# vita-epfl/motion-style-transfer

Measured on AMD Instinct MI355X. Metric: trajectories/sec fwd+bwd (Y-Net+LoRA, SDD shortterm), higher is better.
Workload: dtype f32; 1 GPU; C2: SDD shortterm Y-Net + LoRA rank=1 on encoder[0-4], 256x256 raster, obs=8 pred=12; batch_per_gpu=32, global_batch=32, raster=256x256, obs_len=8, pred_len=12, train_net=mosa_1, parallelism=dp1, trainable_floats=8190

## Files before the change

include/ynet_hip.h:

```cpp
#ifndef YNET_HIP_H
#define YNET_HIP_H

#ifdef __cplusplus
extern "C" {
#endif

int ynet_abi_version(void);
const char* ynet_last_error(void);

long long ynet_packed_weight_floats(int cout, int cin, int K, int mode);
int ynet_pack_weight(const float* w, float* wp, int cout, int cin, int K, int mode, void* stream);

long long ynet_conv2d_workspace_floats(int B, int H, int W, int cout);
int ynet_conv2d(const float* const* src, const int* src_c, const long long* src_bs, const int* src_bmod, int nsrc,
                const float* mask, long long mask_bs, const float* wp, const float* bias,
                float* const* dst, const int* dst_c, const long long* dst_bs, int ndst,
                int B, int H, int W, int K, int relu, float* workspace, long long workspace_floats,
                void* stream);
int ynet_conv2d_pool_supported(int B, int H, int W, int cout, int K);
int ynet_conv2d_pool(const float* const* src, const int* src_c, const long long* src_bs, int nsrc, const float* wp, const float* bias,
                     float* dst, int cout, long long dst_bs, float* pooled, long long pooled_bs,
                     int B, int H, int W, int K, int relu, void* stream);
int ynet_conv2d_dgrad_relu_supported(int B, int H, int W, int dx_c, int K);
int ynet_conv2d_dgrad_relu(const float* dy, int dy_c, long long dy_bs, const float* mask, long long mask_bs, const float* wp,
                           float* dx, int dx_c, long long dx_bs, const float* relu_of, long long relu_of_bs,
                           int B, int H, int W, int K, float* workspace, long long workspace_floats, void* stream);
int ynet_conv2d_add_supported(int B, int H, int W, int cout, int K);
int ynet_conv2d_add(const float* const* src, const int* src_c, const long long* src_bs, const int* src_bmod, int nsrc,
                    const float* wp, const float* bias, float* dst, int cout, long long dst_bs,
                    int B, int H, int W, int K, int relu, const float* addend, long long addend_bs, int addend_bmod,
                    void* stream);

long long ynet_conv2d_relu_bits_words(int B, int H, int W, int cout, int K);
int ynet_conv2d_relu_bits(const float* const* src, const int* src_c, const long long* src_bs, int nsrc, const float* wp, const float* bias,
                          float* dst, int cout, long long dst_bs, unsigned* bits, int B, int H, int W, int K, void* stream);
int ynet_conv2d_dgrad_relu_bits(const float* dy, int dy_c, long long dy_bs, const float* mask, long long mask_bs, const float* wp,
                                float* dx, int dx_c, long long dx_bs, const unsigned* bits, int B, int H, int W, int K, void* stream);

int ynet_conv2d_winograd_supported(int B, int H, int W, int cin, int cout, int K);
long long ynet_winograd_filter_floats(int cin, int cout);
int ynet_winograd_filter(const float* wp, float* u, int cin, int cout, int col0, int cols_total, void* stream);
int ynet_conv2d_winograd(const float* src, long long src_bs, const float* u, const float* bias, float* dst, long long dst_bs, int cin, int cout,
                         int B, int H, int W, int relu, void* stream);
int ynet_conv2d_winograd_s2d(const float* src, long long src_bs, const float* u, float* dst, long long dst_bs, int cin, int cout, int B, int H, int W, void* stream);
int ynet_conv2d_winograd_pred_bce_supported(int B, int H, int W, int cin, int cout, int pred_cout, int kernlen);
int ynet_conv2d_winograd_pred_bce_blob(const float* src, long long src_bs, const float* u, const float* bias, const float* pred_wp, const float* pred_bias, int pred_cout,
                                       const float* target_xy, const float* blob, int kernlen, int S, float* logits, float* loss, float* dx, long long dx_bs,
                                       void* workspace, int B, int H, int W, float expected_grad, void* stream);
int ynet_conv2d_winograd_split_supported(int B, int H, int W, int cin);
int ynet_conv2d_winograd_split(const float* src, long long src_bs, const float* u, float* dst0, long long dst0_bs, int dst0_s2d, float* dst1, long long dst1_bs, int cin,
                               int B, int H, int W, void* stream);
int ynet_conv2d_winograd_dgrad_relu(const float* dy, long long dy_bs, const float* u, float* dx, long long dx_bs, const float* relu_of, long long relu_of_bs,
                                    int dy_c, int dx_c, int B, int H, int W, void* stream);
int ynet_conv2d_winograd_cat_supported(int B, int H, int W, const int* src_c, int nsrc, int cout, int K);
long long ynet_winograd_filter_cat_floats(const int* src_c, int nsrc, int cout);
int ynet_winograd_filter_cat(const float* wp, float* u, const int* src_c, int nsrc, int cout, int col0, int cols_total, void* stream);
int ynet_conv2d_winograd_cat(const float* const* src, const int* src_c, const long long* src_bs, int nsrc, const float* u, const float* bias, float* dst,
                             long long dst_bs, int cout, int B, int H, int W, int relu, void* stream);
int ynet_conv2d_winograd_cat_add(const float* const* src, const int* src_c, const long long* src_bs, int nsrc, const float* u, const float* bias, float* dst,
                                 long long dst_bs, int cout, int B, int H, int W, int relu, const float* addend, long long addend_bs, int addend_bmod,
                                 void* stream);
int ynet_conv2d_winograd_cat_pool(const float* const* src, const int* src_c, const long long* src_bs, int nsrc, const float* u, const float* bias, float* dst,
                                  long long dst_bs, float* pooled, long long pooled_bs, int cout, int B, int H, int W, int relu, void* stream);
int ynet_conv2d_winograd_cat_pool_code(const float* const* src, const int* src_c, const long long* src_bs, int nsrc, const float* u, const float* bias, float* dst,
                                       long long dst_bs, float* pooled, long long pooled_bs, unsigned char* code, int B, int H, int W, void* stream);
long long ynet_winograd_relu_bits_words(int B, int H, int W);
int ynet_conv2d_winograd_relu_bits(const float* src, long long src_bs, const float* u, const float* bias, float* dst, long long dst_bs, int cin, int B, int H, int W,
                                   unsigned* bits_out, void* stream);
int ynet_conv2d_winograd_cat_relu_bits(const float* const* src, const int* src_c, const long long* src_bs, int nsrc, const float* u, const float* bias, float* dst,
                                       long long dst_bs, int B, int H, int W, const float* addend, long long addend_bs, int addend_bmod, unsigned* bits_out,
                                       void* stream);
int ynet_conv2d_winograd_dgrad_relu_bits(const float* dy, long long dy_bs, const float* u, float* dx, long long dx_bs, const unsigned* bits, int dy_c, int B, int H,
                                         int W, void* stream);
int ynet_conv2d_winograd16_supported(int B, int H, int W, const int* src_c, int nsrc, int cout, int K);
long long ynet_winograd16_filter_floats(const int* src_c, int nsrc, int cout);
int ynet_winograd16_filter(const float* wp, float* u, const int* src_c, int nsrc, int cout, int col0, int cols_total, void* stream);
int ynet_conv2d_winograd16(const float* const* src, const int* src_c, const long long* src_bs, int nsrc, const float* u, const float* bias, float* dst,
                           long long dst_bs, int cout, int B, int H, int W, int relu, const float* relu_of, long long relu_of_bs, const float* addend,
                           long long addend_bs, int addend_bmod, float* pooled, long long pooled_bs, void* stream);
int ynet_upsample2x_conv2d_winograd_supported(int B, int H, int W, int cin, int cout, int K);
int ynet_upsample2x_conv2d_winograd(const float* src, long long src_bs, const float* u, const float* bias, float* dst, long long dst_bs, int cin, int cout, int B,
                                    int H, int W, int relu, void* stream);

#define YNET_AUTO_NO_WINOGRAD 1u
#define YNET_AUTO_NO_WINOGRAD16 2u
#define YNET_AUTO_WINOGRAD16_FOR_16 4u
#define YNET_AUTO_NO_POOL_CODE 8u
#define YNET_AUTO_NO_RELU_WBITS 16u
#define YNET_AUTO_NO_SPLIT48 32u
#define YNET_AUTO_UPCONV_BWD 64u
typedef struct YnetConvAuto {
    const float* src[4];
    int src_c[4];
    long long src_bs[4];
    int src_bmod[4];
    int nsrc;
    const float* mask;
    long long mask_bs;
    const float* wp;
    const float* bias;
    float* dst[4];
    int dst_c[4];
    long long dst_bs[4];
    int ndst;
    int B, H, W, K, relu;
    int upsample2x;
    const float* relu_of;
    long long relu_of_bs;
    float* pooled;
    long long pooled_bs;
    unsigned char* pool_code;
    const float* addend;
    long long addend_bs;
    int addend_bmod;
    unsigned* bits_out;
    const unsigned* relu_bits;
    unsigned* wbits_out;
    const unsigned* relu_wbits;
    float* cache;
    long long cache_floats;
    unsigned long long* cache_tag;
    unsigned long long wp_version;
    float* workspace;
    long long workspace_floats;
    unsigned flags;
    int dst_s2d[4];
} YnetConvAuto;
typedef struct YnetConvTaken {
    int family;
    int variant;
    int nlaunch;
    int tmpl[4][3];
    int wrote_wbits, wrote_pool_code, transformed;
    int wrote_s2d;
} YnetConvTaken;
long long ynet_conv2d_auto_cache_floats(const YnetConvAuto* desc);
long long ynet_conv2d_auto_workspace_floats(const YnetConvAuto* desc);
int ynet_conv2d_auto(const YnetConvAuto* desc, YnetConvTaken* taken, void* stream);
int ynet_conv2d_auto_plan(const YnetConvAuto* desc, YnetConvTaken* taken);

long long ynet_upconv_tables_floats(int cout, int cin, long long* keff_floats, long long* table_floats);
int ynet_upconv_tables(const float* w, int cout, int cin, float* keff_packed, float* tables, void* stream);
int ynet_upconv_dgrad_ring(const float* D, long long d_bs, const float* tables, const float* relu_of, long long relu_of_bs, float* dx, long long dx_bs,
                           int B, int C4, int cin, int h, int w, void* stream);

int ynet_conv2d_plan(int B, int H, int W, int cout, int K);

long long ynet_conv2d_wgrad_workspace_floats(int B, int H, int W, int cout, int cin, int K);
int ynet_conv2d_wgrad(const float* const* src, const int* src_c, const long long* src_bs, int nsrc,
                      const float* dy, long long dy_bs, const float* mask, long long mask_bs,
                      float* dw, float* db, float* workspace, int B, int H, int W, int cout, int K,
                      void* stream);

int ynet_lora_compose(const float* w, const float* lora_a, const float* lora_b, float scale, float* w_eff,
                      int cout, int cin, int K, int r, void* stream);
int ynet_lora_grad(const float* dw, const float* lora_a, const float* lora_b, float scale, float* d_a, float* d_b,
                   int cout, int cin, int K, int r, void* stream);

int ynet_lora_compose_pack(const float* w, const float* lora_a, const float* lora_b, float scale, float* wp_fwd,
                           float* wp_dgrad, int cout, int cin, int K, int r, void* stream);
int ynet_lora_compose_pack_multi(int n, const float* const* w, const float* const* lora_a, const float* const* lora_b,
                                 const float* scale, float* const* wp_fwd, float* const* wp_dgrad, const int* cout,
                                 const int* cin, const int* K, const int* r, void* stream);

int ynet_lora_conv2d_wgrad_supported(int cin, int cout, int K, int r, int W);
int ynet_lora_conv2d_wgrad_preferred(int cin, int cout, int K, int r, int W);
long long ynet_lora_conv2d_wgrad_workspace_floats(int cin, int cout);
int ynet_lora_conv2d_wgrad(const float* const* src, const int* src_c, const long long* src_bs, int nsrc,
                           const float* dy, long long dy_batch_stride, const float* mask, long long mask_batch_stride,
                           const float* lora_a, const float* lora_b, float scale, float* d_a, float* d_b,
                           float* workspace, int B, int H, int W, int cout, int K, int r, void* stream);

int ynet_maxpool2_fwd(const float* x, float* y, long long N, int H, int W, void* stream);
int ynet_maxpool2_bwd(const float* x, const float* dy, float* dx, long long N, int H, int W, void* stream);
int ynet_maxpool2_bwd_add(const float* x, const float* dy, const float* add0, const float* add1, float* dx, long long N,
                          int H, int W, int relu_mask, void* stream);
int ynet_maxpool2_bwd_add_code(const unsigned char* code, const float* dy, const float* add0, const float* add1, float* dx, long long N, int H, int W,
                               int relu_mask, void* stream);
int ynet_upsample2x_fwd(const float* x, float* y, long long N, int H, int W, void* stream);
int ynet_upsample2x_bwd(const float* dy, float* dx, long long N, int H, int W, void* stream);
int ynet_upsample2x_bwd_relu(const float* dy, float* dx, const float* relu_of, long long N, int H, int W, void* stream);
int ynet_avgpool_pyramid(const float* x, float* const* outs, int nlev, long long N, int H, int W, void* stream);

long long ynet_batchnorm_workspace_doubles(int C);
int ynet_batchnorm2d_fwd(const float* x, float* y, const float* gamma, const float* beta, float* running_mean, float* running_var, float* save_mean, float* save_invstd,
                         double* workspace, int B, int C, long long HW, int train, double momentum, double eps, void* stream);
int ynet_batchnorm2d_bwd(const float* dy, const float* x, const float* mean, const float* invstd, const float* gamma, float* dx, float* dgamma, float* dbeta, double* workspace,
                         int B, int C, long long HW, int train, void* stream);
int ynet_add_relu(const float* a, const float* b, float* y, long long n, int relu, void* stream);
int ynet_relu_bwd(const float* dy, const float* y, float* dx, long long n, void* stream);

long long ynet_bce_workspace_bytes(void);
int ynet_bce_logits_fwd(const float* x, const float* t, long long n, float* loss, void* workspace, void* stream);
int ynet_bce_logits_bwd(const float* x, const float* t, const float* grad_out, float* dx, long long n, void* stream);
int ynet_bce_logits_fwd_grad(const float* x, const float* t, long long n, float expected_grad, float* loss, float* dx,
                             void* workspace, void* stream);
int ynet_bce_grad_rescale(float* dx, const float* grad_out, float expected_grad, long long n, void* stream);

long long ynet_pred_bce_workspace_bytes(void);
int ynet_pred_bce(const float* x, long long x_batch_stride, const float* wp, const float* bias, const float* target,
                  float* y, float* loss, float* dx, float* dy, void* workspace, int B, int cin, int cout, long long HW,
                  float expected_grad, int dx_relu_mask, void* stream);
int ynet_pred_bce_blob(const float* x, long long x_batch_stride, const float* wp, const float* bias, const float* target_xy, const float* blob, int kernlen,
                       int S, int H, int W, float* y, float* loss, float* dx, float* dy, void* workspace, int B, int cin, int cout, float expected_grad,
                       int dx_relu_mask, void* stream);

int ynet_softargmax2d(const float* x, float* out, long long B, int C, long long batch_stride, int H, int W,
                      void* stream);

// ... 66 lines not shown
```

motion-style-transfer_amd/_lib.py:

```python
import ctypes
import os
import re

_HERE = os.path.dirname(os.path.abspath(__file__))
LIB_PATH = os.environ.get("YNET_HIP_LIB") or os.path.join(_HERE, "csrc", "libynet_hip.so")
HEADER_PATH = os.path.join(os.path.dirname(_HERE), "include", "ynet_hip.h")

c_fp = ctypes.c_void_p
c_i = ctypes.c_int
c_ll = ctypes.c_longlong
c_f = ctypes.c_float
PP = ctypes.POINTER(ctypes.c_void_p)
PI = ctypes.POINTER(ctypes.c_int)
PLL = ctypes.POINTER(ctypes.c_longlong)

class ConvAuto(ctypes.Structure):
    _fields_ = [("src", c_fp * 4), ("src_c", c_i * 4), ("src_bs", c_ll * 4), ("src_bmod", c_i * 4), ("nsrc", c_i),
                ("mask", c_fp), ("mask_bs", c_ll), ("wp", c_fp), ("bias", c_fp),
                ("dst", c_fp * 4), ("dst_c", c_i * 4), ("dst_bs", c_ll * 4), ("ndst", c_i),
                ("B", c_i), ("H", c_i), ("W", c_i), ("K", c_i), ("relu", c_i), ("upsample2x", c_i),
                ("relu_of", c_fp), ("relu_of_bs", c_ll), ("pooled", c_fp), ("pooled_bs", c_ll), ("pool_code", c_fp),
                ("addend", c_fp), ("addend_bs", c_ll), ("addend_bmod", c_i),
                ("bits_out", c_fp), ("relu_bits", c_fp), ("wbits_out", c_fp), ("relu_wbits", c_fp),
                ("cache", c_fp), ("cache_floats", c_ll), ("cache_tag", ctypes.POINTER(ctypes.c_ulonglong)), ("wp_version", ctypes.c_ulonglong),
                ("workspace", c_fp), ("workspace_floats", c_ll), ("flags", ctypes.c_uint), ("dst_s2d", c_i * 4)]


class ConvTaken(ctypes.Structure):
    _fields_ = [("family", c_i), ("variant", c_i), ("nlaunch", c_i), ("tmpl", (c_i * 3) * 4), ("wrote_wbits", c_i), ("wrote_pool_code", c_i),
                ("transformed", c_i), ("wrote_s2d", c_i)]


AUTO_NO_WINOGRAD, AUTO_NO_WINOGRAD16, AUTO_WINOGRAD16_FOR_16, AUTO_NO_POOL_CODE, AUTO_NO_RELU_WBITS, AUTO_NO_SPLIT48 = 1, 2, 4, 8, 16, 32
AUTO_UPCONV_BWD = 64

SIGNATURES = {
    "ynet_abi_version": (c_i, []),
    "ynet_last_error": (ctypes.c_char_p, []),
    "ynet_packed_weight_floats": (c_ll, [c_i, c_i, c_i, c_i]),
    "ynet_pack_weight": (c_i, [c_fp, c_fp, c_i, c_i, c_i, c_i, c_fp]),
    "ynet_conv2d_workspace_floats": (c_ll, [c_i, c_i, c_i, c_i]),
    "ynet_conv2d": (c_i, [PP, PI, PLL, PI, c_i, c_fp, c_ll, c_fp, c_fp, PP, PI, PLL, c_i,
                          c_i, c_i, c_i, c_i, c_i, c_fp, c_ll, c_fp]),
    "ynet_conv2d_pool_supported": (c_i, [c_i, c_i, c_i, c_i, c_i]),
    "ynet_conv2d_pool": (c_i, [PP, PI, PLL, c_i, c_fp, c_fp, c_fp, c_i, c_ll, c_fp, c_ll, c_i, c_i, c_i, c_i, c_i, c_fp]),
    "ynet_conv2d_dgrad_relu_supported": (c_i, [c_i, c_i, c_i, c_i, c_i]),
    "ynet_conv2d_dgrad_relu": (c_i, [c_fp, c_i, c_ll, c_fp, c_ll, c_fp, c_fp, c_i, c_ll, c_fp, c_ll, c_i, c_i, c_i, c_i, c_fp, c_ll, c_fp]),
    "ynet_conv2d_relu_bits_words": (c_ll, [c_i, c_i, c_i, c_i, c_i]),
    "ynet_conv2d_relu_bits": (c_i, [PP, PI, PLL, c_i, c_fp, c_fp, c_fp, c_i, c_ll, c_fp, c_i, c_i, c_i, c_i, c_fp]),
    "ynet_conv2d_dgrad_relu_bits": (c_i, [c_fp, c_i, c_ll, c_fp, c_ll, c_fp, c_fp, c_i, c_ll, c_fp, c_i, c_i, c_i, c_i, c_fp]),
    "ynet_conv2d_winograd_supported": (c_i, [c_i, c_i, c_i, c_i, c_i, c_i]),
    "ynet_winograd_filter_floats": (c_ll, [c_i, c_i]),
    "ynet_winograd_filter": (c_i, [c_fp, c_fp, c_i, c_i, c_i, c_i, c_fp]),
    "ynet_conv2d_winograd": (c_i, [c_fp, c_ll, c_fp, c_fp, c_fp, c_ll, c_i, c_i, c_i, c_i, c_i, c_i, c_fp]),
    "ynet_conv2d_winograd_s2d": (c_i, [c_fp, c_ll, c_fp, c_fp, c_ll, c_i, c_i, c_i, c_i, c_i, c_fp]),
    "ynet_conv2d_winograd_pred_bce_supported": (c_i, [c_i, c_i, c_i, c_i, c_i, c_i, c_i]),
    "ynet_conv2d_winograd_pred_bce_blob": (c_i, [c_fp, c_ll, c_fp, c_fp, c_fp, c_fp, c_i, c_fp, c_fp, c_i, c_i, c_fp, c_fp, c_fp, c_ll, c_fp, c_i, c_i, c_i,
                                                 c_f, c_fp]),
    "ynet_conv2d_winograd_split_supported": (c_i, [c_i, c_i, c_i, c_i]),
    "ynet_conv2d_winograd_split": (c_i, [c_fp, c_ll, c_fp, c_fp, c_ll, c_i, c_fp, c_ll, c_i, c_i, c_i, c_i, c_fp]),
    "ynet_upconv_dgrad_ring": (c_i, [c_fp, c_ll, c_fp, c_fp, c_ll, c_fp, c_ll, c_i, c_i, c_i, c_i, c_i, c_fp]),
    "ynet_upconv_tables_floats": (c_ll, [c_i, c_i, PLL, PLL]),
    "ynet_upconv_tables": (c_i, [c_fp, c_i, c_i, c_fp, c_fp, c_fp]),
    "ynet_conv2d_winograd_dgrad_relu": (c_i, [c_fp, c_ll, c_fp, c_fp, c_ll, c_fp, c_ll, c_i, c_i, c_i, c_i, c_i, c_fp]),
    "ynet_conv2d_winograd_cat_supported": (c_i, [c_i, c_i, c_i, PI, c_i, c_i, c_i]),
    "ynet_winograd_filter_cat_floats": (c_ll, [PI, c_i, c_i]),
    "ynet_winograd_filter_cat": (c_i, [c_fp, c_fp, PI, c_i, c_i, c_i, c_i, c_fp]),
    "ynet_conv2d_winograd_cat": (c_i, [PP, PI, PLL, c_i, c_fp, c_fp, c_fp, c_ll, c_i, c_i, c_i, c_i, c_i, c_fp]),
    "ynet_conv2d_winograd_cat_add": (c_i, [PP, PI, PLL, c_i, c_fp, c_fp, c_fp, c_ll, c_i, c_i, c_i, c_i, c_i, c_fp, c_ll, c_i, c_fp]),
    "ynet_conv2d_winograd_cat_pool": (c_i, [PP, PI, PLL, c_i, c_fp, c_fp, c_fp, c_ll, c_fp, c_ll, c_i, c_i, c_i, c_i, c_i, c_fp]),
    "ynet_conv2d_winograd_cat_pool_code": (c_i, [PP, PI, PLL, c_i, c_fp, c_fp, c_fp, c_ll, c_fp, c_ll, c_fp, c_i, c_i, c_i, c_fp]),
    "ynet_winograd_relu_bits_words": (c_ll, [c_i, c_i, c_i]),
    "ynet_conv2d_winograd_relu_bits": (c_i, [c_fp, c_ll, c_fp, c_fp, c_fp, c_ll, c_i, c_i, c_i, c_i, c_fp, c_fp]),
    "ynet_conv2d_winograd_cat_relu_bits": (c_i, [PP, PI, PLL, c_i, c_fp, c_fp, c_fp, c_ll, c_i, c_i, c_i, c_fp, c_ll, c_i, c_fp, c_fp]),
    "ynet_conv2d_winograd_dgrad_relu_bits": (c_i, [c_fp, c_ll, c_fp, c_fp, c_ll, c_fp, c_i, c_i, c_i, c_i, c_fp]),
    "ynet_upsample2x_conv2d_winograd_supported": (c_i, [c_i, c_i, c_i, c_i, c_i, c_i]),
    "ynet_upsample2x_conv2d_winograd": (c_i, [c_fp, c_ll, c_fp, c_fp, c_fp, c_ll, c_i, c_i, c_i, c_i, c_i, c_i, c_fp]),
    "ynet_conv2d_winograd16_supported": (c_i, [c_i, c_i, c_i, PI, c_i, c_i, c_i]),
    "ynet_winograd16_filter_floats": (c_ll, [PI, c_i, c_i]),
    "ynet_winograd16_filter": (c_i, [c_fp, c_fp, PI, c_i, c_i, c_i, c_i, c_fp]),
    "ynet_conv2d_winograd16": (c_i, [PP, PI, PLL, c_i, c_fp, c_fp, c_fp, c_ll, c_i, c_i, c_i, c_i, c_i, c_fp, c_ll, c_fp, c_ll, c_i, c_fp, c_ll, c_fp]),
    "ynet_conv2d_auto_cache_floats": (c_ll, [ctypes.POINTER(ConvAuto)]),
    "ynet_conv2d_auto_workspace_floats": (c_ll, [ctypes.POINTER(ConvAuto)]),
    "ynet_conv2d_auto": (c_i, [ctypes.POINTER(ConvAuto), ctypes.POINTER(ConvTaken), c_fp]),
    "ynet_conv2d_auto_plan": (c_i, [ctypes.POINTER(ConvAuto), ctypes.POINTER(ConvTaken)]),
    "ynet_conv2d_add_supported": (c_i, [c_i, c_i, c_i, c_i, c_i]),
    "ynet_conv2d_add": (c_i, [PP, PI, PLL, PI, c_i, c_fp, c_fp, c_fp, c_i, c_ll, c_i, c_i, c_i, c_i, c_i, c_fp, c_ll, c_i, c_fp]),
    "ynet_conv2d_plan": (c_i, [c_i, c_i, c_i, c_i, c_i]),
    "ynet_conv2d_wgrad_workspace_floats": (c_ll, [c_i, c_i, c_i, c_i, c_i, c_i]),
    "ynet_conv2d_wgrad": (c_i, [PP, PI, PLL, c_i, c_fp, c_ll, c_fp, c_ll, c_fp, c_fp, c_fp,
                                c_i, c_i, c_i, c_i, c_i, c_fp]),
    "ynet_lora_compose": (c_i, [c_fp, c_fp, c_fp, c_f, c_fp, c_i, c_i, c_i, c_i, c_fp]),
    "ynet_lora_grad": (c_i, [c_fp, c_fp, c_fp, c_f, c_fp, c_fp, c_i, c_i, c_i, c_i, c_fp]),
    "ynet_lora_conv2d_wgrad_supported": (c_i, [c_i, c_i, c_i, c_i, c_i]),
    "ynet_lora_conv2d_wgrad_preferred": (c_i, [c_i, c_i, c_i, c_i, c_i]),
    "ynet_lora_conv2d_wgrad_workspace_floats": (c_ll, [c_i, c_i]),
    "ynet_lora_conv2d_wgrad": (c_i, [PP, PI, PLL, c_i, c_fp, c_ll, c_fp, c_ll, c_fp, c_fp, c_f, c_fp, c_fp, c_fp,
                                     c_i, c_i, c_i, c_i, c_i, c_i, c_fp]),
    "ynet_lora_compose_pack": (c_i, [c_fp, c_fp, c_fp, c_f, c_fp, c_fp, c_i, c_i, c_i, c_i, c_fp]),
    "ynet_lora_compose_pack_multi": (c_i, [c_i, PP, PP, PP, ctypes.POINTER(c_f), PP, PP, PI, PI, PI, PI, c_fp]),
    "ynet_batch_sum": (c_i, [c_fp, c_fp, c_i, c_ll, c_ll, c_fp]),
    "ynet_adam_step": (c_i, [c_fp, c_fp, c_fp, c_i, c_i, ctypes.c_double, ctypes.c_double, ctypes.c_double, ctypes.c_double, ctypes.c_double,
                             c_i, c_fp]),
    "ynet_maxpool2_fwd": (c_i, [c_fp, c_fp, c_ll, c_i, c_i, c_fp]),
    "ynet_maxpool2_bwd": (c_i, [c_fp, c_fp, c_fp, c_ll, c_i, c_i, c_fp]),
    "ynet_maxpool2_bwd_add": (c_i, [c_fp, c_fp, c_fp, c_fp, c_fp, c_ll, c_i, c_i, c_i, c_fp]),
    "ynet_maxpool2_bwd_add_code": (c_i, [c_fp, c_fp, c_fp, c_fp, c_fp, c_ll, c_i, c_i, c_i, c_fp]),
    "ynet_upsample2x_fwd": (c_i, [c_fp, c_fp, c_ll, c_i, c_i, c_fp]),
    "ynet_upsample2x_bwd": (c_i, [c_fp, c_fp, c_ll, c_i, c_i, c_fp]),
    "ynet_upsample2x_bwd_relu": (c_i, [c_fp, c_fp, c_fp, c_ll, c_i, c_i, c_fp]),
    "ynet_avgpool_pyramid": (c_i, [c_fp, PP, c_i, c_ll, c_i, c_i, c_fp]),
    "ynet_bce_workspace_bytes": (c_ll, []),
    "ynet_bce_logits_fwd": (c_i, [c_fp, c_fp, c_ll, c_fp, c_fp, c_fp]),
    "ynet_bce_logits_bwd": (c_i, [c_fp, c_fp, c_fp, c_fp, c_ll, c_fp]),
    "ynet_bce_logits_fwd_grad": (c_i, [c_fp, c_fp, c_ll, c_f, c_fp, c_fp, c_fp, c_fp]),
    "ynet_bce_grad_rescale": (c_i, [c_fp, c_fp, c_f, c_ll, c_fp]),
    "ynet_pred_bce_workspace_bytes": (c_ll, []),
    "ynet_pred_bce": (c_i, [c_fp, c_ll, c_fp, c_fp, c_fp, c_fp, c_fp, c_fp, c_fp, c_fp, c_i, c_i, c_i, c_ll, c_f, c_i, c_fp]),
    "ynet_pred_bce_blob": (c_i, [c_fp, c_ll, c_fp, c_fp, c_fp, c_fp, c_i, c_i, c_i, c_i, c_fp, c_fp, c_fp, c_fp, c_fp, c_i, c_i, c_i, c_f, c_i, c_fp]),
    "ynet_softargmax2d": (c_i, [c_fp, c_fp, c_ll, c_i, c_ll, c_i, c_i, c_fp]),
    "ynet_train_readout": (c_i, [c_fp, c_ll, c_fp, c_ll, c_i, c_fp, c_fp, c_fp, c_fp, c_fp, c_i, c_i, c_i, c_i, c_f, c_fp]),
    "ynet_pred_softargmax_supported": (c_i, [c_i, c_i, c_i, c_i]),
    "ynet_pred_softargmax_workspace_floats": (c_ll, [c_ll, c_i, c_i]),
    "ynet_pred_softargmax": (c_i, [c_fp, c_ll, c_fp, c_fp, c_fp, c_fp, c_ll, c_i, c_i, c_i, c_i, c_fp]),
    "ynet_pad2d": (c_i, [c_fp, c_fp, c_ll, c_i, c_i, c_i, c_i, c_fp]),
    "ynet_seg_onehot_pad": (c_i, [c_fp, c_fp, c_i, c_i, c_i, c_i, c_i, c_fp]),
    "ynet_resize_nearest": (c_i, [c_fp, c_fp, c_i, c_i, c_i, c_i, ctypes.c_double, ctypes.c_double, c_fp]),
    "ynet_batchnorm_workspace_doubles": (c_ll, [c_i]),
    "ynet_batchnorm2d_fwd": (c_i, [c_fp] * 9 + [c_i, c_i, c_ll, c_i, ctypes.c_double, ctypes.c_double, c_fp]),
    "ynet_batchnorm2d_bwd": (c_i, [c_fp] * 9 + [c_i, c_i, c_ll, c_i, c_fp]),
    "ynet_add_relu": (c_i, [c_fp, c_fp, c_fp, c_ll, c_i, c_fp]),
    "ynet_relu_bwd": (c_i, [c_fp, c_fp, c_fp, c_ll, c_fp]),
    "ynet_rot90_flip": (c_i, [c_fp, c_fp, c_ll, c_i, c_i, c_i, c_i, c_fp]),
    "ynet_rot_coords": (c_i, [c_fp, c_ll] + [ctypes.c_double] * 8 + [c_fp]),
    "ynet_sigmoid_temp": (c_i, [c_fp, c_fp, c_ll, c_i, c_ll, PI, c_i, c_f, c_fp]),
    "ynet_gather_patch": (c_i, [c_fp, c_i, c_i, c_fp, c_fp, c_i, c_i, c_i, c_fp, c_fp]),
    "ynet_heatmap_analytic": (c_i, [c_fp, c_fp, c_i, c_i, c_i, c_i, c_i, ctypes.c_double, c_fp, c_i, c_fp, c_fp]),
    "ynet_kmeans2d": (c_i, [c_fp, c_fp, c_fp, c_fp, c_i, c_i, c_i, ctypes.c_float, c_i, c_fp]),
    "ynet_comm_handle_bytes": (c_ll, []),
    "ynet_comm_create": (c_i, [c_i, c_i, c_ll, PP]),
    "ynet_comm_export": (c_i, [c_fp, c_fp]),
    "ynet_comm_connect": (c_i, [c_fp, c_fp]),
    "ynet_allreduce_sum": (c_i, [c_fp, c_fp, c_ll, c_fp]),
    "ynet_comm_status": (c_i, [c_fp]),
    "ynet_comm_destroy": (c_i, [c_fp]),
    "ynet_multinomial": (c_i, [c_fp, c_ll, c_ll, c_i, c_i, c_i, c_f, ctypes.c_ulonglong, c_fp, c_fp, c_fp]),
    "ynet_multinomial_devseed": (c_i, [c_fp, c_ll, c_ll, c_i, c_i, c_i, c_f, c_fp, c_fp, c_fp, c_fp]),
    "ynet_cws_prior": (c_i, [c_fp, c_ll, c_i, c_fp, c_fp, c_i, c_i, c_i, c_f, c_f, c_i, c_fp, c_fp, c_fp]),
    "ynet_score_rank_samples": (c_i, [c_fp, c_fp, c_fp, c_i, c_i, c_i, c_i, c_i, c_i, c_f, c_fp, c_fp, c_fp, c_fp, c_fp, c_fp]),
    "ynet_score_rank_samples_rows": (c_i, [c_fp, c_fp, c_fp, c_fp, c_i, c_i, c_i, c_i, c_i, c_i, c_f, c_fp, c_fp, c_fp, c_fp, c_fp, c_fp]),
    "ynet_gather_rows": (c_i, [c_fp, c_ll, c_fp, c_fp, c_ll, c_i, c_fp, c_fp]),
    "ynet_input_grad_supported": (c_i, [c_i, c_i, c_i, c_i, c_i, c_i]),
    "ynet_input_grad_workspace_floats": (c_ll, [c_i, c_i, c_i, c_i]),
    "ynet_input_grad": (c_i, [c_fp, c_fp, c_fp, c_fp, c_fp, c_fp, c_i, c_i, c_i, c_i, c_i, c_i, c_fp]),
# ... 40 lines not shown
```

motion-style-transfer_amd/csrc/conv_auto.cpp:

```cpp
#include "ynet_common.h"
#include "../../include/ynet_hip.h"
#include <stdint.h>
#include <string.h>

namespace {

struct Piece {
    float* ptr;
    int n;
    long long bs;
    int col0;
    int dst;
    int whole;
};

enum Kind { K_NONE = 0, K_WINO = 1, K_CAT = 2, K_W16 = 3 };

struct Launch {
    int kind;
    int row0;
    int cs[4], ncs;
    int cout, col0, ctot;
    long long floats;
    long long offset;
// ... 17 lines not shown
        case K_CAT: return ynet_winograd_filter_cat_floats(q.cs, q.ncs, q.cout);
        case K_W16: return ynet_winograd16_filter_floats(q.cs, q.ncs, q.cout);
    }
    return 0;
}

void add_launch(Plan& p, int kind, int row0, const int* cs, int ncs, int cout, int col0, int ctot) {
    Launch& q = p.l[p.nl++];
    q.kind = kind;
    q.row0 = row0;
    q.ncs = ncs;
    for (int i = 0; i < 4; ++i) q.cs[i] = i < ncs ? cs[i] : 0;
    q.cout = cout;
    q.col0 = col0;
    q.ctot = ctot;
    q.floats = (filter_floats(q) + 3) & ~3ll;
    q.offset = p.cache_floats;
    p.cache_floats += q.floats;
}

bool w16_ok(const YnetConvAuto* a, const int* cs, int ncs, int cout) {
    return !(a->flags & (YNET_AUTO_NO_WINOGRAD | YNET_AUTO_NO_WINOGRAD16)) && a->K == 3 && ncs >= 1 && ncs <= 3 &&
           ynet_conv2d_winograd16_supported(a->B, a->H, a->W, cs, ncs, cout, a->K);
}

bool srcs_plain(const YnetConvAuto* a) {
    for (int i = 0; i < a->nsrc; ++i)
        if (a->src_bmod[i] > 0) return false;
    return true;
}

bool srcs_aligned(const YnetConvAuto* a) {
    for (int i = 0; i < a->nsrc; ++i)
        if (!al(a->src[i], 16) || (a->src_bs[i] & 3)) return false;
    return true;
}

int make_plan(const YnetConvAuto* a, Plan& p) {
    memset(&p, 0, sizeof(p));
    const bool wino = !(a->flags & YNET_AUTO_NO_WINOGRAD) && a->K == 3 && srcs_plain(a);
    const int B = a->B, H = a->H, W = a->W, K = a->K;
    int cs[4];
    for (int i = 0; i < 4; ++i) cs[i] = i < a->nsrc ? a->src_c[i] : 0;
    int ctot = 0;
    for (int i = 0; i < a->ndst; ++i) ctot += a->dst_c[i];

    if (a->upsample2x) {
        YNET_REQUIRE(a->nsrc == 1 && a->ndst == 1 && !a->mask && !a->relu_of && !a->pooled && !a->addend && !a->bits_out && !a->relu_bits && !a->wbits_out && !a->relu_wbits,
                     "conv2d_auto: upsample2x takes one source, one destination and no other epilogue operand");
        const int s = wino && al(a->src[0], 16) ? ynet_upsample2x_conv2d_winograd_supported(B, H, W, cs[0], ctot, K) : 0;
        YNET_REQUIRE(s == 1 || s == 2, "conv2d_auto: upsample2x + conv is not served for cin %d cout %d at %dx%d (B %d): run ynet_upsample2x_fwd, then the convolution", cs[0], ctot, H, W, B);
        p.family = s == 1 ? 4 : 5;
        add_launch(p, s == 1 ? K_WINO : K_W16, 0, cs, 1, ctot, 0, ctot);
        return 0;
    }
    if (a->bits_out || a->relu_bits) {
        p.family = 0;
        p.variant = a->bits_out ? 1 : 2;
        return 0;
    }
    if (a->addend) {
        YNET_REQUIRE(a->ndst == 1 && !a->mask && !a->relu_of && !a->pooled, "conv2d_auto: addend takes one destination and no mask / relu_of / pooled");
        const bool ok = !(a->flags & YNET_AUTO_NO_WINOGRAD) && K == 3 && srcs_aligned(a) && al(a->addend, 8) && al(a->dst[0], 8) && !(a->dst_bs[0] & 1) && a->nsrc <= 3;
        bool plain = true;
        for (int i = 0; i < a->nsrc; ++i) plain = plain && a->src_bmod[i] <= 0;
        if (ok && plain && ctot == 32 && ynet_conv2d_winograd_cat_supported(B, H, W, cs, a->nsrc, ctot, K)) {
            p.family = 2;
            p.variant = 30;
            add_launch(p, K_CAT, 0, cs, a->nsrc, ctot, 0, ctot);
        } else if (ok && plain && w16_ok(a, cs, a->nsrc, ctot)) {
            p.family = 3;
            p.variant = 31;
            add_launch(p, K_W16, 0, cs, a->nsrc, ctot, 0, ctot);
        } else {
            YNET_REQUIRE(ynet_conv2d_add_supported(B, H, W, ctot, K), "conv2d_auto: a convolution with an additive term is not served at %dx%d (B %d, cout %d, K %d)", H, W, B, ctot, K);
            p.family = 0;
            p.variant = 32;
        }
        return 0;
    }
    if (a->pooled) {
        YNET_REQUIRE(a->ndst == 1 && !a->mask && !a->relu_of, "conv2d_auto: pooled is for a forward convolution with one destination");
        const bool okp = wino && srcs_aligned(a) && al(a->dst[0], 8) && !(a->dst_bs[0] & 1) && a->nsrc <= 3;
        if (okp && ctot == 32 && ynet_conv2d_winograd_cat_supported(B, H, W, cs, a->nsrc, 32, K)) {
            p.family = 2;
            p.variant = 10;
            add_launch(p, K_CAT, 0, cs, a->nsrc, 32, 0, 32);
        } else if (okp && w16_ok(a, cs, a->nsrc, ctot)) {
            p.family = 3;
            p.variant = 11;
            add_launch(p, K_W16, 0, cs, a->nsrc, ctot, 0, ctot);
        } else {
            p.family = 0;
            p.variant = 12;
        }
        return 0;
    }
    if (wino && !a->mask && a->nsrc == 1 && al(a->src[0], 16) && !(a->src_bs[0] & 3) && (!a->relu_of || (al(a->relu_of, 8) && !(a->relu_of_bs & 1)))) {
        const int cin = cs[0];
        const long long HW = (long long)H * W;
        Piece pieces[8];
        int np = 0, c0 = 0;
        bool pieces_ok = true;
        for (int i = 0; i < a->ndst && pieces_ok; ++i) {
            if (!a->dst[i]) { c0 += a->dst_c[i]; continue; }
            int o = 0;
            const int c = a->dst_c[i];
            while (c - o >= 16 && (c - o) % 16 == 0 && np < 8) {
                const int n = c - o >= 32 ? 32 : 16;
                pieces[np++] = Piece{a->dst[i] + o * HW, n, a->dst_bs[i], c0 + o, i, n == c ? 1 : 0};
                o += n;
            }
            if (o != c) pieces_ok = false;
            c0 += c;
        }
        if (!pieces_ok) np = 0;
        auto piece_al = [&](int cnt) {
            for (int i = 0; i < cnt; ++i)
                if (!al(pieces[i].ptr, 8) || (pieces[i].bs & 1)) return false;
            return true;
        };
        if ((a->flags & YNET_AUTO_WINOGRAD16_FOR_16) && np == 1 && pieces[0].n == 16 && piece_al(1) && w16_ok(a, cs, 1, 16)) {
            p.family = 3;
            p.variant = 20;
            p.pieces[0] = pieces[0];
            p.npieces = 1;
            add_launch(p, K_W16, 0, cs, 1, 16, pieces[0].col0, ctot);
            return 0;
        }
        bool wide = false;
        for (int i = 0; i < a->ndst; ++i) wide = wide || (a->dst[i] && a->dst_c[i] >= 64);
        bool all_sup = np > 0 && np <= (a->relu_of ? 1 : 2) && piece_al(np);
        for (int i = 0; i < np && all_sup; ++i) all_sup = ynet_conv2d_winograd_supported(B, H, W, cin, pieces[i].n, K) != 0;
        if (all_sup && !wide && np == 2 && !a->relu_of && !a->bias && !a->relu && !(a->flags & YNET_AUTO_NO_SPLIT48) && pieces[0].n == 16 && pieces[0].whole &&
            pieces[1].n == 32 && pieces[1].whole && pieces[1].col0 == pieces[0].col0 + 16 && ynet_conv2d_winograd_split_supported(B, H, W, cin)) {
            p.family = 1;
            p.variant = 23;
            p.npieces = 2;
            p.pieces[0] = pieces[0];
            p.pieces[1] = pieces[1];
            add_launch(p, K_WINO, 0, cs, 1, 48, pieces[0].col0, ctot);
            return 0;
        }
        if (all_sup && !wide) {
            p.family = 1;
            p.variant = 21;
            p.npieces = np;
            for (int i = 0; i < np; ++i) {
                p.pieces[i] = pieces[i];
                add_launch(p, K_WINO, 0, cs, 1, pieces[i].n, pieces[i].col0, ctot);
            }
            return 0;
        }
        Piece wanted[4];
        int nw = 0;
        c0 = 0;
        for (int i = 0; i < a->ndst; ++i) {
            if (a->dst[i]) wanted[nw++] = Piece{a->dst[i], a->dst_c[i], a->dst_bs[i], c0, i, 1};
            c0 += a->dst_c[i];
        }
        bool w_ok = nw > 0 && (!a->relu_of || nw == 1);
        for (int i = 0; i < nw && w_ok; ++i) w_ok = al(wanted[i].ptr, 8) && !(wanted[i].bs & 1) && w16_ok(a, cs, 1, wanted[i].n);
        if (w_ok) {
            p.family = 3;
            p.variant = 22;
            p.npieces = nw;
// ... 174 lines not shown
        if (a->cache_tag[0] != sig || a->cache_tag[1] != a->wp_version) {
            if (int rc = transform(a, p, stream)) return rc;
            a->cache_tag[0] = sig;
            a->cache_tag[1] = a->wp_version;
            t.transformed = 1;
        }
    }
    return run_plan(a, p, t, taken, stream);
}

}

namespace {

int run_plan(const YnetConvAuto* a, const Plan& p, YnetConvTaken t, YnetConvTaken* taken, void* stream) {
    const int B = a->B, H = a->H, W = a->W, K = a->K, relu = a->relu ? 1 : 0;
    int ctot = 0;
    for (int i = 0; i < a->ndst; ++i) ctot += a->dst_c[i];
    const float* u0 = p.nl ? a->cache + p.l[0].offset : nullptr;
    const float* u1 = p.nl > 1 ? a->cache + p.l[1].offset : nullptr;
    auto done = [&](int rc) {
        if (!rc && taken) *taken = t;
        return rc;
    };
    auto tag = [&](int i, int x, int y, int z) {
        if (i < 4) { t.tmpl[i][0] = x; t.tmpl[i][1] = y; t.tmpl[i][2] = z; }
        t.nlaunch = i + 1;
    };
    float* ws = a->workspace_floats > 0 ? a->workspace : nullptr;
    const long long nws = ws ? a->workspace_floats : 0;

    switch (p.family) {
    case 4:
    case 5:
        tag(0, p.family == 4 ? 4 : 0, 0, 0);
        return done(ynet_upsample2x_conv2d_winograd(a->src[0], a->src_bs[0], u0, a->bias, a->dst[0], a->dst_bs[0], a->src_c[0], ctot, B, H, W, relu, stream));
    case 1: {
        if (p.variant == 23) {
            const Piece &q0 = p.pieces[0], &q1 = p.pieces[1];
            const int s2d = a->dst_s2d[q0.dst] ? 1 : 0;
            const int rc = ynet_conv2d_winograd_split(a->src[0], a->src_bs[0], u0, q0.ptr, q0.bs, s2d, q1.ptr, q1.bs, a->src_c[0], B, H, W, stream);
            if (rc) return rc;
            if (s2d) t.wrote_s2d |= 1 << q0.dst;
            tag(0, 3, a->src_c[0] / 8, s2d ? 6 : 5);
            return done(0);
        }
        const bool one32 = p.npieces == 1 && p.pieces[0].n == 32;
        unsigned* wb_out = (one32 && relu && !a->relu_of && !(a->flags & YNET_AUTO_NO_RELU_WBITS)) ? a->wbits_out : nullptr;
        const unsigned* wb_in = (one32 && a->relu_of && !relu && !a->bias && !(a->flags & YNET_AUTO_NO_RELU_WBITS)) ? a->relu_wbits : nullptr;
        const int em = wb_out ? 3 : (wb_in ? 2 : (a->relu_of ? 1 : 0));
        for (int i = 0; i < p.npieces; ++i) {
            const Piece& q = p.pieces[i];
            const float* u = a->cache + p.l[i].offset;
            const float* bias = a->bias ? a->bias + q.col0 : nullptr;
            int rc;
            const bool s2d = a->dst_s2d[q.dst] && q.whole && em == 0 && !a->bias && !relu;
            if (s2d) {
                rc = ynet_conv2d_winograd_s2d(a->src[0], a->src_bs[0], u, q.ptr, q.bs, a->src_c[0], q.n, B, H, W, stream);
                if (rc) return rc;
                t.wrote_s2d |= 1 << q.dst;
                tag(i, q.n / 16, a->src_c[0] / 8, 4);
                continue;
            }
            if (wb_out) rc = ynet_conv2d_winograd_relu_bits(a->src[0], a->src_bs[0], u, bias, q.ptr, q.bs, a->src_c[0], B, H, W, wb_out, stream);
            else if (wb_in) rc = ynet_conv2d_winograd_dgrad_relu_bits(a->src[0], a->src_bs[0], u, q.ptr, q.bs, wb_in, a->src_c[0], B, H, W, stream);
            else if (a->relu_of) {
                YNET_REQUIRE(!a->bias && !relu, "conv2d_auto: relu_of is for a data gradient (no bias, no ReLU)");
                rc = ynet_conv2d_winograd_dgrad_relu(a->src[0], a->src_bs[0], u, q.ptr, q.bs, a->relu_of, a->relu_of_bs, a->src_c[0], q.n, B, H, W, stream);
            } else rc = ynet_conv2d_winograd(a->src[0], a->src_bs[0], u, bias, q.ptr, q.bs, a->src_c[0], q.n, B, H, W, relu, stream);
            if (rc) return rc;
            tag(i, q.n / 16, a->src_c[0] / 8, em);
        }
        t.wrote_wbits = wb_out ? 1 : 0;
        return done(0);
    }
    case 2: {
        if (p.variant == 30) {
            unsigned* wb = (relu && !(a->flags & YNET_AUTO_NO_RELU_WBITS)) ? a->wbits_out : nullptr;
            tag(0, 2, wb ? 5 : 2, 0);
            t.wrote_wbits = wb ? 1 : 0;
            if (wb) return done(ynet_conv2d_winograd_cat_relu_bits(a->src, a->src_c, a->src_bs, a->nsrc, u0, a->bias, a->dst[0], a->dst_bs[0], B, H, W, a->addend, a->addend_bs, a->addend_bmod, wb, stream));
            return done(ynet_conv2d_winograd_cat_add(a->src, a->src_c, a->src_bs, a->nsrc, u0, a->bias, a->dst[0], a->dst_bs[0], 32, B, H, W, relu, a->addend, a->addend_bs, a->addend_bmod, stream));
        }
        if (p.variant == 10) {
            unsigned char* code = (relu && !(a->flags & YNET_AUTO_NO_POOL_CODE)) ? a->pool_code : nullptr;
            tag(0, 2, code ? 6 : 3, 0);
            t.wrote_pool_code = code ? 1 : 0;
            if (code) return done(ynet_conv2d_winograd_cat_pool_code(a->src, a->src_c, a->src_bs, a->nsrc, u0, a->bias, a->dst[0], a->dst_bs[0], a->pooled, a->pooled_bs, code, B, H, W, stream));
            return done(ynet_conv2d_winograd_cat_pool(a->src, a->src_c, a->src_bs, a->nsrc, u0, a->bias, a->dst[0], a->dst_bs[0], a->pooled, a->pooled_bs, 32, B, H, W, relu, stream));
        }
        unsigned* wb = (relu && !(a->flags & YNET_AUTO_NO_RELU_WBITS)) ? a->wbits_out : nullptr;
        t.wrote_wbits = wb ? 1 : 0;
        if (p.variant == 40) {
            const long long HW = (long long)H * W;
            int rc = ynet_conv2d_winograd(a->src[0], a->src_bs[0], u0, nullptr, a->dst[0], a->dst_bs[0], 32, 32, B, H, W, 0, stream);
            if (rc) return rc;
            const float* rs[4];
            int rc_[4], nr = 0;
            long long rb[4];
            if (a->src_c[0] > 32) { rs[nr] = a->src[0] + 32 * HW; rc_[nr] = a->src_c[0] - 32; rb[nr] = a->src_bs[0]; ++nr; }
            for (int i = 1; i < a->nsrc; ++i) { rs[nr] = a->src[i]; rc_[nr] = a->src_c[i]; rb[nr] = a->src_bs[i]; ++nr; }
            tag(0, 2, 4, 0);
            tag(1, 2, wb ? 5 : 2, 0);
            if (wb) return done(ynet_conv2d_winograd_cat_relu_bits(rs, rc_, rb, nr, u1, a->bias, a->dst[0], a->dst_bs[0], B, H, W, a->dst[0], a->dst_bs[0], 0, wb, stream));
            return done(ynet_conv2d_winograd_cat_add(rs, rc_, rb, nr, u1, a->bias, a->dst[0], a->dst_bs[0], 32, B, H, W, relu, a->dst[0], a->dst_bs[0], 0, stream));
        }
        tag(0, 2, wb ? 4 : 0, 0);
        if (wb) return done(ynet_conv2d_winograd_cat_relu_bits(a->src, a->src_c, a->src_bs, a->nsrc, u0, a->bias, a->dst[0], a->dst_bs[0], B, H, W, nullptr, 0, 0, wb, stream));
        return done(ynet_conv2d_winograd_cat(a->src, a->src_c, a->src_bs, a->nsrc, u0, a->bias, a->dst[0], a->dst_bs[0], 32, B, H, W, relu, stream));
    }
    case 3: {
        if (p.variant == 31) {
            tag(0, 2, 0, 0);
            return done(ynet_conv2d_winograd16(a->src, a->src_c, a->src_bs, a->nsrc, u0, a->bias, a->dst[0], a->dst_bs[0], ctot, B, H, W, relu, nullptr, 0, a->addend, a->addend_bs,
                                               a->addend_bmod, nullptr, 0, stream));
        }
        if (p.variant == 11) {
            tag(0, 3, 0, 0);
            return done(ynet_conv2d_winograd16(a->src, a->src_c, a->src_bs, a->nsrc, u0, a->bias, a->dst[0], a->dst_bs[0], ctot, B, H, W, relu, nullptr, 0, nullptr, 0, 0, a->pooled,
                                               a->pooled_bs, stream));
        }
        if (p.variant == 20 || p.variant == 22) {
            for (int i = 0; i < p.npieces; ++i) {
                const Piece& q = p.pieces[i];
                if (a->relu_of) YNET_REQUIRE(!a->bias && !relu, "conv2d_auto: relu_of is for a data gradient (no bias, no ReLU)");
                int rc = ynet_conv2d_winograd16(a->src, a->src_c, a->src_bs, 1, a->cache + p.l[i].offset, a->bias ? a->bias + q.col0 : nullptr, q.ptr, q.bs, q.n, B, H, W, relu, a->relu_of,
                                                a->relu_of_bs, nullptr, 0, 0, nullptr, 0, stream);
                if (rc) return rc;
                tag(i, a->relu_of ? 1 : 0, 0, 0);
            }
            return done(0);
        }
        if (p.variant == 43) {
            const int cut = p.pieces[0].col0;
            int rc = ynet_conv2d_winograd16(a->src, a->src_c, a->src_bs, cut, u0, nullptr, a->dst[0], a->dst_bs[0], ctot, B, H, W, 0, nullptr, 0, nullptr, 0, 0, nullptr, 0, stream);
            if (rc) return rc;
            tag(0, 0, 0, 0);
            tag(1, 2, 0, 0);
            return done(ynet_conv2d_winograd16(a->src + cut, a->src_c + cut, a->src_bs + cut, a->nsrc - cut, u1, a->bias, a->dst[0], a->dst_bs[0], ctot, B, H, W, relu, nullptr, 0, a->dst[0],
                                               a->dst_bs[0], 0, nullptr, 0, stream));
        }
        tag(0, 0, 0, 0);
        return done(ynet_conv2d_winograd16(a->src, a->src_c, a->src_bs, a->nsrc, u0, a->bias, a->dst[0], a->dst_bs[0], ctot, B, H, W, relu, nullptr, 0, nullptr, 0, 0, nullptr, 0, stream));
    }
    default: break;
    }
    t.nlaunch = 1;
    const int* bmod = nullptr;
    for (int i = 0; i < a->nsrc; ++i)
        if (a->src_bmod[i] > 0) bmod = a->src_bmod;
    switch (p.variant) {
    case 1:
        YNET_REQUIRE(a->ndst == 1 && !a->mask && !a->relu_of && !a->pooled && relu && !bmod, "conv2d_auto: bits_out is for a forward ReLU convolution with one destination");
        return done(ynet_conv2d_relu_bits(a->src, a->src_c, a->src_bs, a->nsrc, a->wp, a->bias, a->dst[0], a->dst_c[0], a->dst_bs[0], a->bits_out, B, H, W, K, stream));
    case 2:
        YNET_REQUIRE(a->nsrc == 1 && a->ndst == 1 && !a->bias && !relu && !a->relu_of, "conv2d_auto: relu_bits is for a data gradient with one source and one destination");
        return done(ynet_conv2d_dgrad_relu_bits(a->src[0], a->src_c[0], a->src_bs[0], a->mask, a->mask_bs, a->wp, a->dst[0], a->dst_c[0], a->dst_bs[0], a->relu_bits, B, H, W, K, stream));
    case 12:
        YNET_REQUIRE(!bmod, "conv2d_auto: pooled takes no batch modulus");
        return done(ynet_conv2d_pool(a->src, a->src_c, a->src_bs, a->nsrc, a->wp, a->bias, a->dst[0], a->dst_c[0], a->dst_bs[0], a->pooled, a->pooled_bs, B, H, W, K, relu, stream));
    case 32:
        return done(ynet_conv2d_add(a->src, a->src_c, a->src_bs, bmod, a->nsrc, a->wp, a->bias, a->dst[0], ctot, a->dst_bs[0], B, H, W, K, relu, a->addend, a->addend_bs, a->addend_bmod, stream));
    case 3:
        YNET_REQUIRE(a->nsrc == 1 && a->ndst == 1 && !a->bias && !relu, "conv2d_auto: relu_of is for a data gradient with one source and one destination");
        return done(ynet_conv2d_dgrad_relu(a->src[0], a->src_c[0], a->src_bs[0], a->mask, a->mask_bs, a->wp, a->dst[0], a->dst_c[0], a->dst_bs[0], a->relu_of, a->relu_of_bs, B, H, W, K, ws,
                                           nws, stream));
// ... 71 lines not shown
```

motion-style-transfer_amd/csrc/conv_wino.hip:

```cpp
#include "ynet_common.h"
#include "bce_element.h"
#include <math.h>
#include <stdlib.h>
#include <type_traits>

typedef float f32x2 __attribute__((ext_vector_type(2)));
typedef unsigned u32x2 __attribute__((ext_vector_type(2)));
typedef __attribute__((address_space(3))) void* lds_ptr_t;

#define WN_TH 16
#define WN_TW 32
#define WN_LQ 10
#define WN_ROWF 40
#define WN_PLANE_F 160
#define WN_SLOT_BYTES (320 * 16 + 16)
#define WN_RING_BYTES (2 * WN_SLOT_BYTES)
#define WN_THREADS 512

struct WinoArgs {
    const float* x;
    const f32x4* u;
    const float* bias;
    float* y;
    long long x_bs, y_bs;
    int B, H, W, relu, ntiles;
    const float* emask;
    long long emask_bs;
    unsigned* wbits;
    float* y2;
    long long y2_bs;
    const float* pw;
    const float* pb;
    int pco, pco_pad;
    const float* t_xy;
    const float* t_blob;
    int t_m, t_S;
    float* logits;
    double* partial;
    unsigned* ticket;
    float* loss;
    long long n_loss;
    float gs;
};

__device__ __forceinline__ f32x2 wn_v01(f32x2 tl, f32x2 th) {
    f32x2 r;
    asm("v_pk_add_f32 %0, %1, %2 op_sel_hi:[1,0] neg_lo:[0,1]" : "=v"(r) : "v"(tl), "v"(th));
    return r;
}
__device__ __forceinline__ f32x2 wn_v23(f32x2 tl, f32x2 th) {
    f32x2 r;
    asm("v_pk_add_f32 %0, %1, %2 op_sel:[1,0] op_sel_hi:[1,1] neg_lo:[1,0] neg_hi:[0,1]" : "=v"(r) : "v"(tl), "v"(th));
    return r;
}

template <int NCB, int EPI, int BITS = 0, bool S2D = false, int CB0 = 0, int CB1 = NCB>
__device__ __forceinline__ void wino_epilogue(f32x4 (&acc)[16][NCB], const f32x2 (&bias2)[NCB][2], float floor_v, __amdgpu_buffer_rsrc_t ry,
                                              __amdgpu_buffer_rsrc_t rm, unsigned st0, unsigned st1, unsigned so_t, unsigned sm_t, int HW, unsigned stp = 0,
                                              unsigned* wbits = nullptr, unsigned char* pcode = nullptr) {
    unsigned word = 0u;
    if constexpr (BITS == 2) word = *wbits;
#pragma unroll
    for (int cb = CB0; cb < CB1; ++cb) {
        constexpr int NB = CB1 - CB0;
        const int cd = cb - CB0;
        u32x2 mk[2][2][2];
        if constexpr (EPI == 1 || EPI == 2) {
#pragma unroll
            for (int h = 0; h < 2; ++h)
#pragma unroll
                for (int k = 0; k < 2; ++k) {
                    const unsigned sm = sm_t + (unsigned)((cd * 16 + 2 * h + k) * HW * 4);
                    mk[h][k][0] = __builtin_amdgcn_raw_buffer_load_b64(rm, st0, sm, 0);
                    mk[h][k][1] = __builtin_amdgcn_raw_buffer_load_b64(rm, st1, sm, 0);
                }
        }
#pragma unroll
        for (int h = 0; h < 2; ++h) {
            f32x2 m[16];
#pragma unroll
            for (int e = 0; e < 16; ++e)
                m[e] = h == 0 ? __builtin_shufflevector(acc[e][cb], acc[e][cb], 0, 1) : __builtin_shufflevector(acc[e][cb], acc[e][cb], 2, 3);
            m[5] = m[5] + bias2[cb][h];
            f32x2 r0[4], r1[4];
#pragma unroll
            for (int j = 0; j < 4; ++j) {
                r0[j] = m[j] + m[4 + j] + m[8 + j];
                r1[j] = m[4 + j] - m[8 + j] - m[12 + j];
            }
            const f32x2 o00 = r0[0] + r0[1] + r0[2], o01 = r0[1] - r0[2] - r0[3];
            const f32x2 o10 = r1[0] + r1[1] + r1[2], o11 = r1[1] - r1[2] - r1[3];
#pragma unroll
            for (int k = 0; k < 2; ++k) {
                f32x2 row0 = {o00[k], o01[k]}, row1 = {o10[k], o11[k]};
                if constexpr (EPI == 2) {
                    row0 += __builtin_bit_cast(f32x2, mk[h][k][0]);
                    row1 += __builtin_bit_cast(f32x2, mk[h][k][1]);
                }
                row0 = f32x2{row0[0] < floor_v ? floor_v : row0[0], row0[1] < floor_v ? floor_v : row0[1]};
                row1 = f32x2{row1[0] < floor_v ? floor_v : row1[0], row1[1] < floor_v ? floor_v : row1[1]};
                if constexpr (EPI == 1) {
                    const f32x2 m0 = __builtin_bit_cast(f32x2, mk[h][k][0]), m1 = __builtin_bit_cast(f32x2, mk[h][k][1]);
                    row0 = f32x2{m0[0] > 0.f ? row0[0] : 0.f, m0[1] > 0.f ? row0[1] : 0.f};
                    row1 = f32x2{m1[0] > 0.f ? row1[0] : 0.f, m1[1] > 0.f ? row1[1] : 0.f};
                }
                const int bit0 = ((cb * 2 + h) * 2 + k) * 4;
                if constexpr (BITS == 2) {
                    row0 = f32x2{(word >> bit0) & 1u ? row0[0] : 0.f, (word >> (bit0 + 1)) & 1u ? row0[1] : 0.f};
                    row1 = f32x2{(word >> (bit0 + 2)) & 1u ? row1[0] : 0.f, (word >> (bit0 + 3)) & 1u ? row1[1] : 0.f};
                }
                if constexpr (BITS == 1)
                    word |= (row0[0] > 0.f ? 1u << bit0 : 0u) | (row0[1] > 0.f ? 2u << bit0 : 0u) | (row1[0] > 0.f ? 4u << bit0 : 0u) | (row1[1] > 0.f ? 8u << bit0 : 0u);
                if constexpr (S2D) {
                    const unsigned hw = (unsigned)(HW >> 2), ph = (unsigned)(NB * 16) * hw * 4u;
                    const unsigned sc = so_t + (unsigned)(cd * 16 + 2 * h + k) * hw * 4u;
                    const float e00 = row0[0], e01 = row0[1], e10 = row1[0], e11 = row1[1];
                    const bool odd = __lane_id() & 1u;
                    const float g0 = __builtin_bit_cast(float, __builtin_amdgcn_update_dpp(0, __builtin_bit_cast(int, odd ? e00 : e01), 0xB1, 0xF, 0xF, false));
                    const float g1 = __builtin_bit_cast(float, __builtin_amdgcn_update_dpp(0, __builtin_bit_cast(int, odd ? e10 : e11), 0xB1, 0xF, 0xF, false));
                    const f32x2 p0 = odd ? f32x2{g0, e01} : f32x2{e00, g0}, p1 = odd ? f32x2{g1, e11} : f32x2{e10, g1};
                    const unsigned vo = st0 + (odd ? ph - 4u : 0u);
                    __builtin_amdgcn_raw_buffer_store_b64(__builtin_bit_cast(u32x2, p0), ry, vo, sc, 0);
                    __builtin_amdgcn_raw_buffer_store_b64(__builtin_bit_cast(u32x2, p1), ry, vo, sc + 2u * ph, 0);
                    continue;
                }
                const unsigned so = so_t + (unsigned)((cd * 16 + 2 * h + k) * HW * 4);
                __builtin_amdgcn_raw_buffer_store_b64(__builtin_bit_cast(u32x2, row0), ry, st0, so, 0);
                __builtin_amdgcn_raw_buffer_store_b64(__builtin_bit_cast(u32x2, row1), ry, st1, so, 0);
                if constexpr (EPI == 3) {
                    float pm = fmaxf(fmaxf(row0[0], row0[1]), fmaxf(row1[0], row1[1]));
                    if (__builtin_isunordered(row0[0], row0[1]) || __builtin_isunordered(row1[0], row1[1])) pm = __builtin_nanf("");
                    __builtin_amdgcn_raw_buffer_store_b32(__builtin_bit_cast(unsigned, pm), rm, stp, sm_t + (unsigned)((cd * 16 + 2 * h + k) * (HW >> 2) * 4), 0);
                    if constexpr (BITS == 3) {
                        float mx = row0[0];
                        unsigned arg = 0u;
                        if (row0[1] > mx || row0[1] != row0[1]) { mx = row0[1]; arg = 1u; }
                        if (row1[0] > mx || row1[0] != row1[0]) { mx = row1[0]; arg = 2u; }
                        if (row1[1] > mx || row1[1] != row1[1]) { mx = row1[1]; arg = 3u; }
                        const unsigned code = arg | (row0[0] > 0.f ? 4u : 0u) | (row0[1] > 0.f ? 8u : 0u) | (row1[0] > 0.f ? 16u : 0u) | (row1[1] > 0.f ? 32u : 0u);
                        pcode[(cd * 16 + 2 * h + k) * (HW >> 2)] = (unsigned char)code;
                    }
                }
            }
        }
    }
    if constexpr (BITS == 1) *wbits = word;
}

template <int MB, typename PosT>
__device__ __forceinline__ float wino_epilogue_pred(f32x4 (&acc)[16][2], const f32x2 (&bias2)[2][2], const f32x4* tab,
                                                    const WinoArgs& a, __amdgpu_buffer_rsrc_t rdx, __amdgpu_buffer_rsrc_t rlog, unsigned st_rm, unsigned so_rm, int b,
                                                    int py0, int px0, int kq, int H, int W, const float* blob_tab, const PosT* pos_lds) {
    const int HW = H * W;
    float yv[2][4][4];
#pragma unroll
    for (int cb = 0; cb < 2; ++cb)
#pragma unroll
        for (int h = 0; h < 2; ++h) {
            f32x2 m[16];
#pragma unroll
            for (int e = 0; e < 16; ++e)
                m[e] = h == 0 ? __builtin_shufflevector(acc[e][cb], acc[e][cb], 0, 1) : __builtin_shufflevector(acc[e][cb], acc[e][cb], 2, 3);
            m[5] = m[5] + bias2[cb][h];
            f32x2 r0[4], r1[4];
#pragma unroll
            for (int j = 0; j < 4; ++j) {
                r0[j] = m[j] + m[4 + j] + m[8 + j];
                r1[j] = m[4 + j] - m[8 + j] - m[12 + j];
            }
            const f32x2 o00 = r0[0] + r0[1] + r0[2], o01 = r0[1] - r0[2] - r0[3];
            const f32x2 o10 = r1[0] + r1[1] + r1[2], o11 = r1[1] - r1[2] - r1[3];
#pragma unroll
            for (int k = 0; k < 2; ++k) {
                const float v00 = o00[k], v01 = o01[k], v10 = o10[k], v11 = o11[k];
                yv[cb][2 * h + k][0] = v00 < 0.f ? 0.f : v00;
                yv[cb][2 * h + k][1] = v01 < 0.f ? 0.f : v01;
                yv[cb][2 * h + k][2] = v10 < 0.f ? 0.f : v10;
                yv[cb][2 * h + k][3] = v11 < 0.f ? 0.f : v11;
            }
        }
    const unsigned st1 = st_rm + (unsigned)(W * 4);
    float s = 0.f;
    f32x4 dx[2][4];
#pragma unroll
    for (int cb = 0; cb < 2; ++cb)
#pragma unroll
        for (int p = 0; p < 4; ++p) dx[cb][p] = f32x4{0.f, 0.f, 0.f, 0.f};
    auto block = [&](const int mb) {
        f32x4 z[4], dz[4];
        {
            const f32x4 pbv = tab[(4 * MB + mb) * 64];
#pragma unroll
            for (int p = 0; p < 4; ++p) z[p] = pbv;
        }
#pragma unroll
        for (int cb = 0; cb < 2; ++cb) {
            const f32x4 wa = tab[(mb * 2 + cb) * 64];
#pragma unroll
            for (int j = 0; j < 4; ++j)
#pragma unroll
                for (int p = 0; p < 4; ++p) z[p] = __builtin_amdgcn_mfma_f32_16x16x4f32(wa[j], yv[cb][j][p], z[p], 0, 0, 0);
        }
#pragma unroll
        for (int i = 0; i < 4; ++i) {
            const int o = 16 * mb + 4 * kq + i;
            const bool valid = o < a.pco;
            const int rx = valid ? (int)pos_lds[2 * (b * a.pco + o)] : 32767, ry = valid ? (int)pos_lds[2 * (b * a.pco + o) + 1] : 32767;
#pragma unroll
            for (int p = 0; p < 4; ++p) {
                const int by = py0 + (p >> 1) - ry + a.t_m / 2, bx = px0 + (p & 1) - rx + a.t_m / 2;
#if defined(YNET_PRED_EPI_DIAG) && (YNET_PRED_EPI_DIAG & 2)
                const float t = 0.f;
#else
                const float t = (by >= 0 && by < a.t_m && bx >= 0 && bx < a.t_m) ? blob_tab[by * a.t_m + bx] : 0.f;
#endif
                float de;
#if defined(YNET_PRED_EPI_DIAG) && (YNET_PRED_EPI_DIAG & 1)
                de = (z[p][i] - t) * a.gs;
                const float l = z[p][i] - t;
#else
                const float l = bce_element<true, true>(z[p][i], t, a.gs, de);
#endif
                s += valid ? l : 0.f;
                dz[p][i] = valid ? de : 0.f;
            }
        }
#pragma unroll
        for (int i = 0; i < 4; ++i) {
            const f32x2 row0 = {z[0][i], z[1][i]}, row1 = {z[2][i], z[3][i]};
            const unsigned so = so_rm + (unsigned)((16 * mb + i) * HW * 4);
            __builtin_amdgcn_raw_buffer_store_b64(__builtin_bit_cast(u32x2, row0), rlog, st_rm, so, 0);
// ... 265 lines not shown
                cur = nxt;
                if (cur < total_units) nxt = next_unit();
                continue;
            }
            if constexpr (EM == 5 || EM == 6) {
                static_assert(EM < 5 || NCB == 3, "the two-destination epilogue is the 48-channel launch's");
                const __amdgpu_buffer_rsrc_t r0 = __builtin_amdgcn_make_buffer_rsrc(a.y + (long long)b * a.y_bs, 0, (unsigned)(16 * HW * 4), 0x00020000);
                const __amdgpu_buffer_rsrc_t r1 = __builtin_amdgcn_make_buffer_rsrc(a.y2 + (long long)b * a.y2_bs, 0, (unsigned)(32 * HW * 4), 0x00020000);
                if constexpr (EM == 6) wino_epilogue<NCB, 0, 0, true, 0, 1>(acc, bias2, floor_v, r0, r0, st_s2d, st_s2d, so_s2d, so_s2d, HW);
                else wino_epilogue<NCB, 0, 0, false, 0, 1>(acc, bias2, floor_v, r0, r0, st_rm, st_rm + (unsigned)(W * 4), so_rm, so_rm, HW);
                wino_epilogue<NCB, 0, 0, false, 1, 3>(acc, bias2, floor_v, r1, r1, st_rm, st_rm + (unsigned)(W * 4), so_rm, so_rm, HW);
                cur = nxt;
                if (cur < total_units) nxt = next_unit();
                continue;
            }
            const unsigned so_t = EM == 4 ? so_s2d : so_rm;
            const __amdgpu_buffer_rsrc_t ry = __builtin_amdgcn_make_buffer_rsrc(a.y + (long long)b * a.y_bs, 0, y_img, 0x00020000);
            const __amdgpu_buffer_rsrc_t rm =
                __builtin_amdgcn_make_buffer_rsrc(const_cast<float*>(EM == 1 ? a.emask + (long long)b * a.emask_bs : a.y), 0, y_img, 0x00020000);
            unsigned* wb = (EM == 2 || EM == 3) ? a.wbits + (((long long)b * (H >> 1) + (ty * (WN_TH / 2) + (cur & 7))) * tiles_x + tx) * 64 + lane : nullptr;
            wino_epilogue<NCB, EM == 1 ? 1 : 0, EM == 2 ? 2 : (EM == 3 ? 1 : 0), EM == 4>(acc, bias2, floor_v, ry, rm, st0, st1, so_t, so_t, HW, 0, wb);
        }
        cur = nxt;
        if (cur < total_units) nxt = next_unit();
    }
    if constexpr (EM == 7 || EM == 8) {
        double* wsd = reinterpret_cast<double*>(ptab + 5 * PMB * 64);
        unsigned* last = reinterpret_cast<unsigned*>(wsd + NW);
#pragma unroll
        for (int o = 32; o > 0; o >>= 1) acc_loss += __shfl_xor(acc_loss, o, 64);
        if (lane == 0) wsd[wave] = acc_loss;
        __syncthreads();
        if (tid == 0) {
            double t = 0.0;
            for (int i = 0; i < NW; ++i) t += wsd[i];
            a.partial[blockIdx.x] = t;
            __threadfence();
            *last = (atomicAdd(a.ticket, 1u) == gridDim.x - 1) ? 1u : 0u;
        }
        __syncthreads();
        if (*last) {
            __threadfence();
            double t = 0.0;
            for (unsigned i = tid; i < gridDim.x; i += NT) t += ((volatile double*)a.partial)[i];
#pragma unroll
            for (int o = 32; o > 0; o >>= 1) t += __shfl_xor(t, o, 64);
            if (lane == 0) wsd[wave] = t;
            __syncthreads();
            if (tid == 0) {
                double tt = 0.0;
                for (int i = 0; i < NW; ++i) tt += wsd[i];
                a.loss[0] = (float)(tt / (double)a.n_loss);
                *a.ticket = 0u;
            }
        }
    }
}

#define WC_SLOT_BYTES (160 * 16 + 16)
#define WC_RING_BYTES (2 * WC_SLOT_BYTES)
#define WC_MAX_SRC 3

struct WinoCatArgs {
    const float* x[WC_MAX_SRC];
    long long x_bs[WC_MAX_SRC];
    int x_c[WC_MAX_SRC];
    int nsrc, nchunks;
    const f32x4* u;
    const float* bias;
    float* y;
    long long y_bs;
    int B, H, W, relu, ntiles;
    const float* addend;
    long long addend_bs;
    int addend_bmod;
    float* pool;
    long long pool_bs;
    unsigned char* pcode;
    unsigned* wbits;
};

template <int NCB, int EPI_>
__global__ __launch_bounds__(WN_THREADS, 1) void conv_wino_cat_kernel(const WinoCatArgs a) {
    constexpr int EPI = EPI_ == 4 ? 0 : (EPI_ == 5 ? 2 : (EPI_ == 6 ? 3 : EPI_));
    constexpr int BITS = EPI_ == 6 ? 3 : (EPI_ >= 4 ? 1 : 0);
    constexpr bool ADD = EPI == 2;
    extern __shared__ f32x4 smem[];
    constexpr int WQ = 4 * NCB * 64;
    const int tid = threadIdx.x, lane = tid & 63;
    const int wave = __builtin_amdgcn_readfirstlane(tid >> 6);
    const int H = a.H, W = a.W, HW = H * W, nchunks = a.nchunks;
    const int tiles_x = W / WN_TW, tiles_y = H / WN_TH;
    const unsigned lds0 = __builtin_amdgcn_readfirstlane((unsigned)(uintptr_t)smem);
    const unsigned wbytes = (unsigned)(nchunks * WQ * 16);
    const unsigned ring0 = lds0 + wbytes + (unsigned)(wave * WC_RING_BYTES);

    unsigned rel[3], edge[3], planeof[3];
#pragma unroll
    for (int j = 0; j < 3; ++j) {
        const int u = j * 64 + lane, plane = u / 40, rem = u - plane * 40, r = rem / WN_LQ, xq = rem - r * WN_LQ;
        rel[j] = (unsigned)((plane * HW + r * W + 4 * xq) * 4);
        edge[j] = (r == 0 ? 1u : 0u) | (r == 3 ? 2u : 0u) | (xq == 0 ? 4u : 0u) | (xq == WN_LQ - 1 ? 8u : 0u);
        planeof[j] = (unsigned)plane;
    }
    const unsigned lead = (unsigned)((W + 4) * 4);
    const __amdgpu_buffer_rsrc_t ru = __builtin_amdgcn_make_buffer_rsrc(const_cast<f32x4*>(a.u), 0, wbytes, 0x00020000);
    const unsigned y_img = (unsigned)(NCB * 16 * HW * 4);

    const bool xcd_walk = (gridDim.x & 7) == 0 && a.ntiles >= (int)gridDim.x;
    const int per_xcd = (a.ntiles + 7) >> 3;
    const int gstride = xcd_walk ? (int)(gridDim.x >> 3) : (int)gridDim.x;
    const int tile_first = xcd_walk ? (int)(blockIdx.x & 7) * per_xcd + (int)(blockIdx.x >> 3) : (int)blockIdx.x;
    const int tile_end = xcd_walk ? min(a.ntiles, ((int)(blockIdx.x & 7) + 1) * per_xcd) : a.ntiles;
    if (tile_first >= tile_end) return;
    const int my_tiles = (tile_end - tile_first + gstride - 1) / gstride;
    const int total_units = my_tiles * 8;

    const int n = lane & 15, kq = lane >> 4;
    const float floor_v = a.relu ? 0.f : -INFINITY;
    f32x2 bias2[NCB][2];
#pragma unroll
    for (int cb = 0; cb < NCB; ++cb)
#pragma unroll
        for (int h = 0; h < 2; ++h)
            bias2[cb][h] = a.bias ? f32x2{a.bias[cb * 16 + 4 * kq + 2 * h], a.bias[cb * 16 + 4 * kq + 2 * h + 1]} : f32x2{0.f, 0.f};
    asm volatile("s_waitcnt vmcnt(0)" ::: "memory");
#pragma unroll
    for (int cb = 0; cb < NCB; ++cb)
#pragma unroll
        for (int h = 0; h < 2; ++h) asm volatile("" : "+v"(bias2[cb][h]));
    const unsigned st0 = (unsigned)((4 * kq * HW + 2 * n) * 4), st1 = st0 + (unsigned)(W * 4);
    const unsigned stp = (unsigned)((4 * kq * (HW >> 2) + n) * 4);

    for (int j = 0; j < nchunks * WQ / WN_THREADS; ++j)
        __builtin_amdgcn_raw_ptr_buffer_load_lds(ru, (lds_ptr_t)(uintptr_t)(lds0 + (unsigned)(j * 8192 + wave * 1024)), 16,
                                                 (unsigned)((j * WN_THREADS + tid) * 16), 0, 0, 0);
    unsigned* unit_ctr = reinterpret_cast<unsigned*>(reinterpret_cast<unsigned char*>(smem) + wbytes + 8 * WC_RING_BYTES);
    if (tid == 0) *unit_ctr = 8u;
    asm volatile("s_waitcnt vmcnt(0) lgkmcnt(0)" ::: "memory");
    asm volatile("s_barrier" ::: "memory");
    auto next_unit = [&]() {
        unsigned u = 0;
        if (lane == 0) u = atomicAdd(unit_ctr, 1u);
        return (int)__builtin_amdgcn_readfirstlane(u);
    };

    auto dma_chunk = [&](int unit, int c, int slot) {
        const int t = tile_first + (unit >> 3) * gstride;
        const int tx = t % tiles_x, ty = (t / tiles_x) % tiles_y, b = t / (tiles_x * tiles_y);
        const int y0 = ty * WN_TH + 2 * (unit & 7), x0 = tx * WN_TW;
        const unsigned em = (y0 == 0 ? 1u : 0u) | (y0 + 2 == H ? 2u : 0u) | (x0 == 0 ? 4u : 0u) | (x0 + WN_TW == W ? 8u : 0u);
        int s = 0, ch = c * 4;
        while (s + 1 < a.nsrc && ch >= ((a.x_c[s] + 3) & ~3)) {
            ch -= (a.x_c[s] + 3) & ~3;
            ++s;
        }
        const unsigned nvalid = (unsigned)min(4, a.x_c[s] - ch);
        const __amdgpu_buffer_rsrc_t rx = __builtin_amdgcn_make_buffer_rsrc(
            const_cast<unsigned char*>(reinterpret_cast<const unsigned char*>(a.x[s] + (long long)b * a.x_bs[s]) - lead), 0,
            (unsigned)(a.x_c[s] * HW * 4) + lead, 0x00020000);
        const unsigned so = (unsigned)((ch * HW + y0 * W + x0) * 4);
        const unsigned sb = ring0 + (unsigned)(slot * WC_SLOT_BYTES) + 4u;
        if (em == 0 && nvalid == 4) {
            __builtin_amdgcn_raw_ptr_buffer_load_lds(rx, (lds_ptr_t)(uintptr_t)sb, 16, rel[0], so, 0, 0);
            __builtin_amdgcn_raw_ptr_buffer_load_lds(rx, (lds_ptr_t)(uintptr_t)(sb + 1024u), 16, rel[1], so, 0, 0);
            if (lane < 32) __builtin_amdgcn_raw_ptr_buffer_load_lds(rx, (lds_ptr_t)(uintptr_t)(sb + 2048u), 16, rel[2], so, 0, 0);
        } else {
            const unsigned v0 = ((edge[0] & em) || planeof[0] >= nvalid) ? 0x80000000u : rel[0];
            const unsigned v1 = ((edge[1] & em) || planeof[1] >= nvalid) ? 0x80000000u : rel[1];
            const unsigned v2 = ((edge[2] & em) || planeof[2] >= nvalid) ? 0x80000000u : rel[2];
            __builtin_amdgcn_raw_ptr_buffer_load_lds(rx, (lds_ptr_t)(uintptr_t)sb, 16, v0, so, 0, 0);
            __builtin_amdgcn_raw_ptr_buffer_load_lds(rx, (lds_ptr_t)(uintptr_t)(sb + 1024u), 16, v1, so, 0, 0);
            if (lane < 32) __builtin_amdgcn_raw_ptr_buffer_load_lds(rx, (lds_ptr_t)(uintptr_t)(sb + 2048u), 16, v2, so, 0, 0);
        }
    };

    int cur = wave, nxt = next_unit();
    int g = 0;
    dma_chunk(cur, 0, 0);
    dma_chunk(cur, 1, 1);

    f32x4 acc[16][NCB];
    const unsigned char* ringp = reinterpret_cast<const unsigned char*>(smem) + wbytes + wave * WC_RING_BYTES;
    while (cur < total_units) {
        auto step = [&](int c, auto first) {
            if (c + 1 < nchunks || nxt < total_units) asm volatile("s_waitcnt vmcnt(3)" ::: "memory");
            else asm volatile("s_waitcnt vmcnt(0)" ::: "memory");
            const int slot = g & 1;
            const float* ip = reinterpret_cast<const float*>(ringp + slot * WC_SLOT_BYTES + 4) + kq * WN_PLANE_F + 3 + 2 * n;
            f32x2 dl[4], dh[4];
#pragma unroll
            for (int r = 0; r < 4; ++r) {
                dl[r] = *reinterpret_cast<const f32x2*>(ip + r * WN_ROWF);
                dh[r] = *reinterpret_cast<const f32x2*>(ip + r * WN_ROWF + 2);
            }
            asm volatile("s_waitcnt lgkmcnt(0)" ::: "memory");
            if (c + 2 < nchunks) dma_chunk(cur, c + 2, slot);
            else if (nxt < total_units) dma_chunk(nxt, c + 2 - nchunks, slot);
            wino_kstep<NCB, decltype(first)::value>(acc, dl, dh, smem + c * WQ, lane);
            ++g;
        };
        step(0, std::true_type{});
        for (int c = 1; c < nchunks; ++c) step(c, std::false_type{});
        {
            const int t = tile_first + (cur >> 3) * gstride;
            const int tx = t % tiles_x, ty = (t / tiles_x) % tiles_y, b = t / (tiles_x * tiles_y);
            const unsigned so_t = (unsigned)(((ty * WN_TH + 2 * (cur & 7)) * W + tx * WN_TW) * 4);
            const int ab = a.addend_bmod > 0 ? b % a.addend_bmod : b;
            const unsigned sa_t = EPI == 3 ? (unsigned)(((ty * (WN_TH / 2) + (cur & 7)) * (W >> 1) + tx * (WN_TW / 2)) * 4) : so_t;
            const __amdgpu_buffer_rsrc_t ry = __builtin_amdgcn_make_buffer_rsrc(a.y + (long long)b * a.y_bs, 0, y_img, 0x00020000);
            const __amdgpu_buffer_rsrc_t ra =
                EPI == 3 ? __builtin_amdgcn_make_buffer_rsrc(a.pool + (long long)b * a.pool_bs, 0, y_img >> 2, 0x00020000)
                         : __builtin_amdgcn_make_buffer_rsrc(const_cast<float*>(ADD ? a.addend + (long long)ab * a.addend_bs : a.y), 0, y_img, 0x00020000);
            unsigned* wb = BITS == 1 ? a.wbits + (((long long)b * (H >> 1) + (ty * (WN_TH / 2) + (cur & 7))) * tiles_x + tx) * 64 + lane : nullptr;
            unsigned char* pc = BITS == 3 ? a.pcode + ((long long)b * (16 * NCB) * (HW >> 2) + ((stp + sa_t) >> 2)) : nullptr;
            wino_epilogue<NCB, EPI, BITS>(acc, bias2, floor_v, ry, ra, st0, st1, so_t, sa_t, HW, stp, wb, pc);
        }
        cur = nxt;
        if (cur < total_units) nxt = next_unit();
    }
}

#define W6_PLANE_BYTES 1152
#define W6_SLOT_BYTES (4 * W6_PLANE_BYTES + 16)
#define W6_RING_BYTES (2 * W6_SLOT_BYTES)
#define W6_MAX_CHUNKS 21
#define W6_TH 32

struct Wino16Args {
    const float* x[WC_MAX_SRC];
    long long x_bs[WC_MAX_SRC];
    int x_c[WC_MAX_SRC];
    int nsrc, nchunks;
    const f32x4* u;
    const float* bias;
    float* y;
    long long y_bs;
    int ns;
    int B, H, W, relu, ntiles;
    const float* aux;
    long long aux_bs;
    int aux_bmod;
    float* pool;
    long long pool_bs;
};

template <bool FIRST>
__device__ __forceinline__ void wino16_kstep(f32x4 (&acc)[2][16][1], const f32x2 (&dl)[6], const f32x2 (&dh)[6], const f32x4* wl, int lane) {
    f32x2 v01[2][4], v23[2][4];
#pragma unroll
    for (int p = 0; p < 2; ++p) {
        const f32x2 tl[4] = {dl[2 * p] - dl[2 * p + 2], dl[2 * p + 1] + dl[2 * p + 2], dl[2 * p + 2] - dl[2 * p + 1], dl[2 * p + 1] - dl[2 * p + 3]};
        const f32x2 th[4] = {dh[2 * p] - dh[2 * p + 2], dh[2 * p + 1] + dh[2 * p + 2], dh[2 * p + 2] - dh[2 * p + 1], dh[2 * p + 1] - dh[2 * p + 3]};
#pragma unroll
        for (int i = 0; i < 4; ++i) {
            v01[p][i] = wn_v01(tl[i], th[i]);
            v23[p][i] = wn_v23(tl[i], th[i]);
        }
    }
    asm volatile("s_nop 3"
                 : "+v"(v01[0][0]), "+v"(v01[0][1]), "+v"(v01[0][2]), "+v"(v01[0][3]), "+v"(v23[0][0]), "+v"(v23[0][1]), "+v"(v23[0][2]), "+v"(v23[0][3]),
                   "+v"(v01[1][0]), "+v"(v01[1][1]), "+v"(v01[1][2]), "+v"(v01[1][3]), "+v"(v23[1][0]), "+v"(v23[1][1]), "+v"(v23[1][2]), "+v"(v23[1][3]));
#pragma unroll
    for (int q = 0; q < 4; ++q) {
        const f32x4 w = wl[q * 64 + lane];
#pragma unroll
        for (int e = 0; e < 4; ++e) {
#pragma unroll
            for (int p = 0; p < 2; ++p) {
                const float bv = e < 2 ? v01[p][q][e] : v23[p][q][e - 2];
                if constexpr (FIRST) acc[p][q * 4 + e][0] = __builtin_amdgcn_mfma_f32_16x16x4f32(w[e], bv, f32x4{0.f, 0.f, 0.f, 0.f}, 0, 0, 0);
                else acc[p][q * 4 + e][0] = __builtin_amdgcn_mfma_f32_16x16x4f32(w[e], bv, acc[p][q * 4 + e][0], 0, 0, 0);
            }
        }
    }
}

template <int EPI>
__global__ __launch_bounds__(WN_THREADS, 1) void conv_wino16_kernel(const Wino16Args a) {
    extern __shared__ f32x4 smem[];
    constexpr int WQ = 4 * 64;
    const int tid = threadIdx.x, lane = tid & 63;
    const int wave = __builtin_amdgcn_readfirstlane(tid >> 6);
    const int H = a.H, W = a.W, HW = H * W, nchunks = a.nchunks;
    const int tiles_x = W / WN_TW, tiles_y = H / W6_TH;
    const unsigned lds0 = __builtin_amdgcn_readfirstlane((unsigned)(uintptr_t)smem);
    const unsigned wbytes = (unsigned)(nchunks * WQ * 16);
    const unsigned ring0 = lds0 + wbytes + (unsigned)(wave * W6_RING_BYTES);

    const int r6 = lane / WN_LQ, xq = lane - r6 * WN_LQ;
    const unsigned rel = (unsigned)((r6 * W + 4 * xq) * 4);
    const unsigned edge = (r6 == 0 ? 1u : 0u) | (r6 == 5 ? 2u : 0u) | (xq == 0 ? 4u : 0u) | (xq == WN_LQ - 1 ? 8u : 0u);
    const unsigned lead = (unsigned)((W + 4) * 4);
    const unsigned y_img = (unsigned)(16 * HW * 4);

    const int g8 = (int)(gridDim.x >> 3), idx = (int)(blockIdx.x >> 3);
    const int slice = idx % a.ns, gstride = g8 / a.ns;
    const int per_xcd = (a.ntiles + 7) >> 3;
    const int tile_first = (int)(blockIdx.x & 7) * per_xcd + idx / a.ns;
// ... 466 lines not shown
    for (int t = 0; t < 9; ++t) g[t / 3][t % 3] = row >= 0 ? wp[((long long)row * 9 + t) * cols_pad + co] : 0.f;
    float gr[3];
#pragma unroll
    for (int j = 0; j < 3; ++j)
        gr[j] = q == 0 ? g[0][j] : (q == 3 ? g[2][j] : 0.5f * ((g[0][j] + g[2][j]) + (q == 1 ? g[1][j] : -g[1][j])));
    f32x4 o;
    o[0] = gr[0];
    o[1] = 0.5f * ((gr[0] + gr[2]) + gr[1]);
    o[2] = 0.5f * ((gr[0] + gr[2]) - gr[1]);
    o[3] = gr[2];
    u[i] = o;
}

static int wino_cols_pad(int cols) { return ceil_div(cols, 64) * 64; }

static bool wino_shape_ok(int B, int H, int W, int cin, int cout, int K) {
    static const int on = getenv("YNET_WINOGRAD") ? atoi(getenv("YNET_WINOGRAD")) : 1;
    if (!on || K != 3 || B <= 0) return false;
    if (H % WN_TH || W % WN_TW || H < WN_TH || W < WN_TW) return false;
    static const int on48 = getenv("YNET_WINOGRAD48") ? atoi(getenv("YNET_WINOGRAD48")) : 1;
    if ((cin != 16 && cin != 32) || (cout != 16 && cout != 32 && !(cout == 48 && on48))) return false;
    if (48ll * H * W * 4 + (W + 4) * 4 >= (1ll << 31)) return false;
    static const int min_pixels = getenv("YNET_WINOGRAD_MIN") ? atoi(getenv("YNET_WINOGRAD_MIN")) : 128 * 128 * 8;
    return (long long)B * H * W >= min_pixels;
}

template <int NCB, int NCH, int EM, int NW>
static int launch_wino_nw(WinoArgs& a, hipStream_t st) {
    const int lds = NCH * 8 * NCB * 64 * 16 + NW * WN_RING_BYTES + 16 +
                    (EM == 7 ? 5 * 64 * 16 + NW * 8 + 16 + (a.t_m * a.t_m + 2 * a.B * a.pco) * 4
                             : (EM == 8 ? 10 * 64 * 16 + NW * 8 + 16 + a.t_m * a.t_m * 4 + ((2 * a.B * a.pco * 2 + 15) & ~15) : 0));
    static bool attr_dev[YNET_MAX_DEV] = {false};
    static int cus_dev[YNET_MAX_DEV] = {0};
    const int slot = ynet_device_slot();
    if (!attr_dev[slot]) {
        (void)hipFuncSetAttribute(reinterpret_cast<const void*>(conv_wino_kernel<NCB, NCH, EM, NW>), hipFuncAttributeMaxDynamicSharedMemorySize, (EM == 7 || EM == 8) ? 160 * 1024 : lds);
        int dev = 0, cus = 256;
        (void)hipGetDevice(&dev);
        (void)hipDeviceGetAttribute(&cus, hipDeviceAttributeMultiprocessorCount, dev);
        cus_dev[slot] = cus < 8 ? 8 : cus;
        attr_dev[slot] = true;
    }
    int grid = a.ntiles < cus_dev[slot] ? a.ntiles : cus_dev[slot];
    if (grid >= 8) grid &= ~7;
    hipLaunchKernelGGL((conv_wino_kernel<NCB, NCH, EM, NW>), dim3(grid), dim3(NW * 64), lds, st, a);
    return ynet_check_launch("conv2d_winograd");
}

template <int NCB, int NCH, int EM>
static int launch_wino(WinoArgs& a, hipStream_t st) {
    static const int w12 = getenv("YNET_WINOGRAD_W12") ? atoi(getenv("YNET_WINOGRAD_W12")) : 0;
    if constexpr (NCB == 1) {
        if (w12) return launch_wino_nw<NCB, NCH, EM, 12>(a, st);
    }
    return launch_wino_nw<NCB, NCH, EM, 8>(a, st);
}

extern "C" {

int ynet_conv2d_winograd_supported(int B, int H, int W, int cin, int cout, int K) { return wino_shape_ok(B, H, W, cin, cout, K) ? 1 : 0; }

long long ynet_winograd_filter_floats(int cin, int cout) {
    if (cin <= 0 || cout <= 0) return 0;
    return 16ll * (ceil_div(cin, 8) * 8) * (ceil_div(cout, 16) * 16);
}

int ynet_winograd_filter(const float* wp, float* u, int cin, int cout, int col0, int cols_total, void* stream) {
    YNET_REQUIRE(wp && u, "winograd_filter: null pointer");
    YNET_REQUIRE(cin > 0 && cin % 8 == 0 && cout > 0 && cout % 16 == 0, "winograd_filter: cin %d must be a multiple of 8, cout %d of 16", cin, cout);
    YNET_REQUIRE(col0 >= 0 && cols_total >= col0 + cout, "winograd_filter: output channels %d .. %d are not inside the filter's %d", col0, col0 + cout, cols_total);
    YNET_REQUIRE((reinterpret_cast<uintptr_t>(u) & 15) == 0, "winograd_filter: the output must be 16-byte aligned");
    const int ncb = cout / 16, nunits = (cin / 4) * 4 * ncb * 64;
    hipLaunchKernelGGL(wino_filter_kernel, dim3(ceil_div(nunits, 256)), dim3(256), 0, (hipStream_t)stream, wp, reinterpret_cast<f32x4*>(u),
                       wino_cols_pad(cols_total), col0, ncb, nunits, cin, 0, 0, 0);
    return ynet_check_launch("winograd_filter");
}

static int wino_cat_padded(const int* src_c, int nsrc) {
    int n = 0;
    for (int i = 0; i < nsrc; ++i) n += (src_c[i] + 3) & ~3;
    return n;
}

static bool wino_cat_ok(int B, int H, int W, const int* src_c, int nsrc, int cout, int K) {
    static const int on = getenv("YNET_WINOGRAD") ? atoi(getenv("YNET_WINOGRAD")) : 1;
    static const int cat_on = getenv("YNET_WINOGRAD_CAT") ? atoi(getenv("YNET_WINOGRAD_CAT")) : 1;
    if (!on || !cat_on || K != 3 || B <= 0 || nsrc < 1 || nsrc > WC_MAX_SRC || cout != 32) return false;
    if (H % WN_TH || W % WN_TW || H < WN_TH || W < WN_TW) return false;
    for (int i = 0; i < nsrc; ++i)
        if (src_c[i] <= 0) return false;
    const int nch = wino_cat_padded(src_c, nsrc) / 4;
    if (56ll * H * W * 4 + (W + 4) * 4 >= (1ll << 31)) return false;
    if (nch < 2 || nch > 14) return false;
    static const int min_pixels = getenv("YNET_WINOGRAD_MIN") ? atoi(getenv("YNET_WINOGRAD_MIN")) : 128 * 128 * 8;
    return (long long)B * H * W >= min_pixels;
}

int ynet_conv2d_winograd_cat_supported(int B, int H, int W, const int* src_c, int nsrc, int cout, int K) {
    return (src_c != nullptr && wino_cat_ok(B, H, W, src_c, nsrc, cout, K)) ? 1 : 0;
}

long long ynet_winograd_filter_cat_floats(const int* src_c, int nsrc, int cout) {
    if (src_c == nullptr || nsrc < 1 || nsrc > WC_MAX_SRC || cout <= 0) return 0;
    return 16ll * wino_cat_padded(src_c, nsrc) * (ceil_div(cout, 16) * 16);
}

int ynet_winograd_filter_cat(const float* wp, float* u, const int* src_c, int nsrc, int cout, int col0, int cols_total, void* stream) {
    YNET_REQUIRE(wp && u && src_c, "winograd_filter_cat: null pointer");
    YNET_REQUIRE(nsrc >= 1 && nsrc <= WC_MAX_SRC && cout > 0 && cout % 16 == 0, "winograd_filter_cat: 1..%d sources, cout %d a multiple of 16", WC_MAX_SRC, cout);
    YNET_REQUIRE(col0 >= 0 && cols_total >= col0 + cout, "winograd_filter_cat: output channels %d .. %d are not inside the filter's %d", col0, col0 + cout, cols_total);
    YNET_REQUIRE((reinterpret_cast<uintptr_t>(u) & 15) == 0, "winograd_filter_cat: the output must be 16-byte aligned");
    for (int i = 0; i < nsrc; ++i) YNET_REQUIRE(src_c[i] > 0, "winograd_filter_cat: source %d has no channels", i);
    const int ncb = cout / 16, nunits = wino_cat_padded(src_c, nsrc) * ncb * 64;
    hipLaunchKernelGGL(wino_filter_kernel, dim3(ceil_div(nunits, 256)), dim3(256), 0, (hipStream_t)stream, wp, reinterpret_cast<f32x4*>(u),
                       wino_cols_pad(cols_total), col0, ncb, nunits, src_c[0], nsrc > 1 ? src_c[1] : 0, nsrc > 2 ? src_c[2] : 0, 0);
    return ynet_check_launch("winograd_filter_cat");
}

static int wino_cat_launch(const float* const* src, const int* src_c, const long long* src_bs, int nsrc, const float* u, const float* bias, float* dst,
                           long long dst_bs, int cout, int B, int H, int W, int relu, const float* addend, long long addend_bs, int addend_bmod, float* pool,
                           long long pool_bs, void* stream, const char* what, unsigned* wbits = nullptr, unsigned char* pcode = nullptr) {
    YNET_REQUIRE(src && src_c && src_bs && u && dst, "%s: null pointer", what);
    YNET_REQUIRE(wino_cat_ok(B, H, W, src_c, nsrc, cout, 3), "%s: shape B=%d %dx%d -> %d with %d sources is not served (ask ynet_conv2d_winograd_cat_supported)", what,
                 B, H, W, cout, nsrc);
    const long long HW = (long long)H * W;
    WinoCatArgs a{};
    for (int i = 0; i < nsrc; ++i) {
        YNET_REQUIRE(src[i] != nullptr && (reinterpret_cast<uintptr_t>(src[i]) & 15) == 0 && (src_bs[i] & 3) == 0 && (src_bs[i] == 0 || src_bs[i] >= src_c[i] * HW),
                     "%s: source %d must be 16-byte aligned with a batch stride of 0 (one image for the batch) or not smaller than its image", what, i);
        a.x[i] = src[i];
        a.x_bs[i] = src_bs[i];
        a.x_c[i] = src_c[i];
    }
    YNET_REQUIRE((reinterpret_cast<uintptr_t>(dst) & 7) == 0 && (reinterpret_cast<uintptr_t>(u) & 15) == 0 && (dst_bs & 1) == 0 && dst_bs >= cout * HW,
                 "%s: the output must be 8-byte aligned, its batch stride not smaller than the image", what);
    if (addend != nullptr) {
        YNET_REQUIRE(addend_bmod >= 0 && (reinterpret_cast<uintptr_t>(addend) & 7) == 0 && (addend_bs & 1) == 0 && addend_bs >= cout * HW,
                     "%s: the additive term must be 8-byte aligned, its image stride not smaller than the image, its modulus not negative", what);
    }
    if (pool != nullptr)
        YNET_REQUIRE(addend == nullptr && (reinterpret_cast<uintptr_t>(pool) & 3) == 0 && pool_bs >= cout * (HW / 4),
                     "%s: the pooled copy must have a batch stride not smaller than its image, and excludes an additive term", what);
    if (wbits != nullptr)
        YNET_REQUIRE(pool == nullptr && (reinterpret_cast<uintptr_t>(wbits) & 3) == 0, "%s: the 1-bit mask excludes the pooled copy and must be 4-byte aligned", what);
    if (pcode != nullptr) YNET_REQUIRE(pool != nullptr && cout == 32 && relu, "%s: the arg-max / ReLU bytes come with the pooled copy of a 32-channel ReLU output", what);
    a.wbits = wbits;
    a.pool = pool;
    a.pool_bs = pool_bs;
    a.pcode = pcode;
    a.nsrc = nsrc;
    a.nchunks = wino_cat_padded(src_c, nsrc) / 4;
    a.u = reinterpret_cast<const f32x4*>(u);
    a.bias = bias;
    a.y = dst;
    a.y_bs = dst_bs;
    a.B = B; a.H = H; a.W = W; a.relu = relu ? 1 : 0;
    a.ntiles = B * (H / WN_TH) * (W / WN_TW);
    a.addend = addend;
    a.addend_bs = addend_bs;
    a.addend_bmod = addend_bmod;
    const int lds = a.nchunks * 8192 + 8 * WC_RING_BYTES + 16;
    static bool attr_dev[YNET_MAX_DEV] = {false};
    static int cus_dev[YNET_MAX_DEV] = {0};
    const int slot = ynet_device_slot();
    if (!attr_dev[slot]) {
        (void)hipFuncSetAttribute(reinterpret_cast<const void*>(conv_wino_cat_kernel<2, 0>), hipFuncAttributeMaxDynamicSharedMemorySize, 14 * 8192 + 8 * WC_RING_BYTES + 16);
        (void)hipFuncSetAttribute(reinterpret_cast<const void*>(conv_wino_cat_kernel<2, 2>), hipFuncAttributeMaxDynamicSharedMemorySize, 14 * 8192 + 8 * WC_RING_BYTES + 16);
        (void)hipFuncSetAttribute(reinterpret_cast<const void*>(conv_wino_cat_kernel<2, 3>), hipFuncAttributeMaxDynamicSharedMemorySize, 14 * 8192 + 8 * WC_RING_BYTES + 16);
        (void)hipFuncSetAttribute(reinterpret_cast<const void*>(conv_wino_cat_kernel<2, 4>), hipFuncAttributeMaxDynamicSharedMemorySize, 14 * 8192 + 8 * WC_RING_BYTES + 16);
        (void)hipFuncSetAttribute(reinterpret_cast<const void*>(conv_wino_cat_kernel<2, 5>), hipFuncAttributeMaxDynamicSharedMemorySize, 14 * 8192 + 8 * WC_RING_BYTES + 16);
        (void)hipFuncSetAttribute(reinterpret_cast<const void*>(conv_wino_cat_kernel<2, 6>), hipFuncAttributeMaxDynamicSharedMemorySize, 14 * 8192 + 8 * WC_RING_BYTES + 16);
        int dev = 0, cus = 256;
        (void)hipGetDevice(&dev);
        (void)hipDeviceGetAttribute(&cus, hipDeviceAttributeMultiprocessorCount, dev);
        cus_dev[slot] = cus < 8 ? 8 : cus;
        attr_dev[slot] = true;
    }
    int grid = a.ntiles < cus_dev[slot] ? a.ntiles : cus_dev[slot];
    if (grid >= 8) grid &= ~7;
    if (wbits != nullptr && addend != nullptr) hipLaunchKernelGGL((conv_wino_cat_kernel<2, 5>), dim3(grid), dim3(WN_THREADS), lds, (hipStream_t)stream, a);
    else if (wbits != nullptr) hipLaunchKernelGGL((conv_wino_cat_kernel<2, 4>), dim3(grid), dim3(WN_THREADS), lds, (hipStream_t)stream, a);
    else if (addend != nullptr) hipLaunchKernelGGL((conv_wino_cat_kernel<2, 2>), dim3(grid), dim3(WN_THREADS), lds, (hipStream_t)stream, a);
    else if (pcode != nullptr) hipLaunchKernelGGL((conv_wino_cat_kernel<2, 6>), dim3(grid), dim3(WN_THREADS), lds, (hipStream_t)stream, a);
    else if (pool != nullptr) hipLaunchKernelGGL((conv_wino_cat_kernel<2, 3>), dim3(grid), dim3(WN_THREADS), lds, (hipStream_t)stream, a);
    else hipLaunchKernelGGL((conv_wino_cat_kernel<2, 0>), dim3(grid), dim3(WN_THREADS), lds, (hipStream_t)stream, a);
    return ynet_check_launch(what);
}

int ynet_conv2d_winograd_cat(const float* const* src, const int* src_c, const long long* src_bs, int nsrc, const float* u, const float* bias, float* dst,
                             long long dst_bs, int cout, int B, int H, int W, int relu, void* stream) {
    return wino_cat_launch(src, src_c, src_bs, nsrc, u, bias, dst, dst_bs, cout, B, H, W, relu, nullptr, 0, 0, nullptr, 0, stream, "conv2d_winograd_cat");
}

int ynet_conv2d_winograd_cat_add(const float* const* src, const int* src_c, const long long* src_bs, int nsrc, const float* u, const float* bias, float* dst,
                                 long long dst_bs, int cout, int B, int H, int W, int relu, const float* addend, long long addend_bs, int addend_bmod,
                                 void* stream) {
    YNET_REQUIRE(addend != nullptr, "conv2d_winograd_cat_add: the additive term is null");
    return wino_cat_launch(src, src_c, src_bs, nsrc, u, bias, dst, dst_bs, cout, B, H, W, relu, addend, addend_bs, addend_bmod, nullptr, 0, stream, "conv2d_winograd_cat_add");
}

int ynet_conv2d_winograd_cat_pool(const float* const* src, const int* src_c, const long long* src_bs, int nsrc, const float* u, const float* bias, float* dst,
                                  long long dst_bs, float* pooled, long long pooled_bs, int cout, int B, int H, int W, int relu, void* stream) {
    YNET_REQUIRE(pooled != nullptr, "conv2d_winograd_cat_pool: the pooled output is null");
    return wino_cat_launch(src, src_c, src_bs, nsrc, u, bias, dst, dst_bs, cout, B, H, W, relu, nullptr, 0, 0, pooled, pooled_bs, stream, "conv2d_winograd_cat_pool");
}

int ynet_conv2d_winograd_cat_pool_code(const float* const* src, const int* src_c, const long long* src_bs, int nsrc, const float* u, const float* bias, float* dst,
                                       long long dst_bs, float* pooled, long long pooled_bs, unsigned char* code, int B, int H, int W, void* stream) {
    YNET_REQUIRE(pooled != nullptr && code != nullptr, "conv2d_winograd_cat_pool_code: the pooled output or its code plane is null");
    return wino_cat_launch(src, src_c, src_bs, nsrc, u, bias, dst, dst_bs, 32, B, H, W, 1, nullptr, 0, 0, pooled, pooled_bs, stream, "conv2d_winograd_cat_pool_code",
                           nullptr, code);
}

static int wino_launch_any(const float* src, long long src_bs, const float* u, const float* bias, float* dst, long long dst_bs, const float* emask,
                           long long emask_bs, int cin, int cout, int B, int H, int W, int relu, void* stream, const char* what, unsigned* wbits = nullptr,
                           bool wbits_apply = false, bool s2d = false, float* dst2 = nullptr, long long dst2_bs = 0, int split_mode = 0) {
    YNET_REQUIRE(src && u && dst, "%s: null pointer", what);
    YNET_REQUIRE(wino_shape_ok(B, H, W, cin, cout, 3), "%s: shape B=%d %dx%d %d -> %d is not served (ask ynet_conv2d_winograd_supported)", what, B, H, W, cin,
                 cout);
    YNET_REQUIRE((reinterpret_cast<uintptr_t>(src) & 15) == 0 && (reinterpret_cast<uintptr_t>(dst) & 7) == 0 && (reinterpret_cast<uintptr_t>(u) & 15) == 0 &&
                     (src_bs & 3) == 0 && (dst_bs & 1) == 0,
                 "%s: planes must be 16-byte (input, filters) / 8-byte (output) aligned", what);
    const long long HW = (long long)H * W;
    YNET_REQUIRE((src_bs == 0 || src_bs >= cin * HW) && dst_bs >= (split_mode ? 16 : cout) * HW, "%s: batch strides smaller than the images (input: 0 = one image for the batch)", what);
    if (split_mode)
        YNET_REQUIRE(cout == 48 && dst2 != nullptr && (reinterpret_cast<uintptr_t>(dst2) & 7) == 0 && (dst2_bs & 1) == 0 && dst2_bs >= 32 * HW && bias == nullptr && !relu &&
                         wbits == nullptr && !s2d,
                     "%s: two destinations are for the plain 48-channel data gradient (16 + 32 planes, 8-byte aligned)", what);
    if (emask != nullptr)
        YNET_REQUIRE((reinterpret_cast<uintptr_t>(emask) & 7) == 0 && (emask_bs & 1) == 0 && emask_bs >= cout * HW,
                     "%s: the activation must be 8-byte aligned, its batch stride not smaller than the image", what);
    WinoArgs a{src, reinterpret_cast<const f32x4*>(u), bias, dst, src_bs, dst_bs, B, H, W, relu ? 1 : 0, B * (H / WN_TH) * (W / WN_TW), emask, emask_bs, wbits, dst2, dst2_bs};
    hipStream_t st = (hipStream_t)stream;
    if (wbits != nullptr) {
        YNET_REQUIRE(cout == 32 && emask == nullptr && (reinterpret_cast<uintptr_t>(wbits) & 3) == 0, "%s: the 1-bit mask serves 32 output channels and excludes the float mask", what);
        if (wbits_apply) return cin == 32 ? launch_wino<2, 4, 2>(a, st) : launch_wino<2, 2, 2>(a, st);
        return cin == 32 ? launch_wino<2, 4, 3>(a, st) : launch_wino<2, 2, 3>(a, st);
    }
    if (s2d) {
        YNET_REQUIRE(emask == nullptr && bias == nullptr && !relu, "%s: the space-to-depth store is for a plain data gradient", what);
        if (cout == 32) return cin == 32 ? launch_wino<2, 4, 4>(a, st) : launch_wino<2, 2, 4>(a, st);
        return cin == 32 ? launch_wino<1, 4, 4>(a, st) : launch_wino<1, 2, 4>(a, st);
    }
    if (cout == 48) {
        YNET_REQUIRE(emask == nullptr && cin == 32, "%s: the 48-channel form is plain, from 32 input channels", what);
        if (split_mode == 1) return launch_wino_nw<3, 4, 5, 4>(a, st);
        if (split_mode == 2) return launch_wino_nw<3, 4, 6, 4>(a, st);
        return launch_wino_nw<3, 4, 0, 4>(a, st);
    }
    if (emask != nullptr) {
        if (cout == 32) return cin == 32 ? launch_wino<2, 4, 1>(a, st) : launch_wino<2, 2, 1>(a, st);
        return cin == 32 ? launch_wino<1, 4, 1>(a, st) : launch_wino<1, 2, 1>(a, st);
    }
    if (cout == 32) return cin == 32 ? launch_wino<2, 4, 0>(a, st) : launch_wino<2, 2, 0>(a, st);
    return cin == 32 ? launch_wino<1, 4, 0>(a, st) : launch_wino<1, 2, 0>(a, st);
}

int ynet_conv2d_winograd(const float* src, long long src_bs, const float* u, const float* bias, float* dst, long long dst_bs, int cin, int cout,
                         int B, int H, int W, int relu, void* stream) {
    return wino_launch_any(src, src_bs, u, bias, dst, dst_bs, nullptr, 0, cin, cout, B, H, W, relu, stream, "conv2d_winograd");
}

int ynet_conv2d_winograd_s2d(const float* src, long long src_bs, const float* u, float* dst, long long dst_bs, int cin, int cout, int B, int H, int W, void* stream) {
    return wino_launch_any(src, src_bs, u, nullptr, dst, dst_bs, nullptr, 0, cin, cout, B, H, W, 0, stream, "conv2d_winograd_s2d", nullptr, false, true);
}

int ynet_conv2d_winograd_pred_bce_supported(int B, int H, int W, int cin, int cout, int pred_cout, int kernlen) {
    static const int on = getenv("YNET_CONV_PRED_BCE") ? atoi(getenv("YNET_CONV_PRED_BCE")) : 1;
    if (!(on && cin == 32 && cout == 32 && pred_cout >= 1 && pred_cout <= 32 && kernlen >= 1 && wino_shape_ok(B, H, W, cin, cout, 3))) return 0;
    const long long base = 4ll * 8 * 2 * 64 * 16 + 8ll * WN_RING_BYTES + 16 + 8 * 8 + 16;
    const long long lds = pred_cout <= 16 ? base + 5 * 64 * 16 + ((long long)kernlen * kernlen + 2ll * B * pred_cout) * 4
                                          : base + 10 * 64 * 16 + (long long)kernlen * kernlen * 4 + ((2ll * B * pred_cout * 2 + 15) & ~15ll);
    return lds <= 160 * 1024 ? 1 : 0;
}

int ynet_conv2d_winograd_pred_bce_blob(const float* src, long long src_bs, const float* u, const float* bias, const float* pred_wp, const float* pred_bias, int pred_cout,
                                       const float* target_xy, const float* blob, int kernlen, int S, float* logits, float* loss, float* dx, long long dx_bs,
                                       void* workspace, int B, int H, int W, float expected_grad, void* stream) {
    YNET_REQUIRE(src && u && pred_wp && target_xy && blob && logits && loss && dx && workspace, "conv2d_winograd_pred_bce_blob: null pointer");
    YNET_REQUIRE(ynet_conv2d_winograd_pred_bce_supported(B, H, W, 32, 32, pred_cout, kernlen), "conv2d_winograd_pred_bce_blob: B=%d %dx%d with %d predictor outputs and a %d x %d blob is not served (32 -> 32, <= 32 outputs, tables within LDS; ask ..._supported)",
                 B, H, W, pred_cout, kernlen, kernlen);
    YNET_REQUIRE(kernlen > 0 && kernlen <= S && S >= H && S >= W, "conv2d_winograd_pred_bce_blob: the target needs a blob table with 0 < kernlen <= S and S >= H, W (got kernlen %d, S %d, %dx%d)", kernlen, S, H, W);
    const long long HW = (long long)H * W;
    YNET_REQUIRE((reinterpret_cast<uintptr_t>(src) & 15) == 0 && (reinterpret_cast<uintptr_t>(u) & 15) == 0 && (reinterpret_cast<uintptr_t>(dx) & 7) == 0 &&
                     (reinterpret_cast<uintptr_t>(logits) & 7) == 0 && (src_bs & 3) == 0 && (dx_bs & 1) == 0 && (src_bs == 0 || src_bs >= 32 * HW) && dx_bs >= 32 * HW,
                 "conv2d_winograd_pred_bce_blob: planes must be 16-byte (input, filters) / 8-byte (outputs) aligned, batch strides not smaller than the images");
    WinoArgs a{src, reinterpret_cast<const f32x4*>(u), bias, dx, src_bs, dx_bs, B, H, W, 1, B * (H / WN_TH) * (W / WN_TW), nullptr, 0, nullptr, nullptr, 0};
    a.pw = pred_wp;
    a.pb = pred_bias;
    a.pco = pred_cout;
    a.pco_pad = ceil_div(pred_cout, 64) * 64;
    a.t_xy = target_xy;
    a.t_blob = blob;
    a.t_m = kernlen;
// ... 237 lines not shown
```

motion-style-transfer_amd/ops.py:

```python
import ctypes
from typing import List, Sequence

import numpy as np
import torch

from . import _lib as L

MAX_SRC = 4
_VP = ctypes.c_void_p


def _lib():
    return L.load()


def _stream():
    return _VP(torch.cuda.current_stream().cuda_stream)


def _need_gpu(t: torch.Tensor, what: str, dtypes=(torch.float32,)):
    if not torch.is_tensor(t):
        raise TypeError(f"{what}: expected a torch.Tensor, got {type(t)}")
    if not t.is_cuda:
        raise RuntimeError(f"{what}: tensor is on {t.device}; the MI355X path runs on HIP devices only "
# ... 284 lines not shown
wino_stats = {"launches": 0}
_wino_eval_min_hw = 0
_wino_cat_eval = True
_wino_plain_eval = True


def _wino_made(entry):
    if not torch.cuda.is_available() or torch.cuda.is_current_stream_capturing():
        return entry + (None, None)
    ev = torch.cuda.Event()
    ev.record()
    return entry + (torch.cuda.current_stream().cuda_stream, ev)


def _wino_ready(entry):
    stream, ev = entry[-2], entry[-1]
    if ev is not None and not torch.cuda.is_current_stream_capturing():
        cur = torch.cuda.current_stream()
        if cur.cuda_stream != stream and not ev.query():
            cur.wait_event(ev)
    return entry


def winograd_filter(wp: torch.Tensor, cin: int, cout: int, col0: int = 0, cols_total: int = None) -> torch.Tensor:
    lib = _lib()
    u = torch.empty(lib.ynet_winograd_filter_floats(cin, cout), device=wp.device, dtype=torch.float32)
    L.check(lib.ynet_winograd_filter(wp.data_ptr(), u.data_ptr(), cin, cout, col0, cout if cols_total is None else cols_total, _stream()), lib)
    return u


def conv2d_winograd_raw(src, u, bias, dst, cin, cout, B, H, W, relu, relu_of=None, wbits_out=None, relu_wbits=None, s2d=False):
    lib = _lib()
    if s2d:
        if bias is not None or relu or relu_of is not None or wbits_out is not None or relu_wbits is not None:
            raise ValueError("conv2d_winograd_raw: s2d is for a plain data gradient")
        L.check(lib.ynet_conv2d_winograd_s2d(src[0], src[1], u.data_ptr(), dst[0], dst[1], cin, cout, B, H, W, _stream()), lib)
        return
    if wbits_out is not None:
        if cout != 32 or not relu or relu_of is not None or relu_wbits is not None:
            raise ValueError("conv2d_winograd_raw: wbits_out is for a forward ReLU launch with 32 outputs")
        L.check(lib.ynet_conv2d_winograd_relu_bits(src[0], src[1], u.data_ptr(), bias.data_ptr() if bias is not None else None, dst[0], dst[1], cin, B, H, W,
                                                   wbits_out.data_ptr(), _stream()), lib)
        return
    if relu_wbits is not None:
        if cout != 32 or bias is not None or relu or relu_of is not None:
            raise ValueError("conv2d_winograd_raw: relu_wbits is for a data gradient with 32 outputs")
        L.check(lib.ynet_conv2d_winograd_dgrad_relu_bits(src[0], src[1], u.data_ptr(), dst[0], dst[1], relu_wbits.data_ptr(), cin, B, H, W, _stream()), lib)
        return
    if relu_of is not None:
        if bias is not None or relu:
            raise ValueError("conv2d_winograd_raw: relu_of is for a data gradient")
        L.check(lib.ynet_conv2d_winograd_dgrad_relu(src[0], src[1], u.data_ptr(), dst[0], dst[1], relu_of[0], relu_of[1], cin, cout, B, H, W, _stream()), lib)
        return
    L.check(lib.ynet_conv2d_winograd(src[0], src[1], u.data_ptr(), bias.data_ptr() if bias is not None else None, dst[0], dst[1],
                                     cin, cout, B, H, W, 1 if relu else 0, _stream()), lib)


def conv2d_winograd_pred_bce_raw(src, u, bias, pred_wp, pred_bias, pred_cout, pos, tmpl, logits, loss, dx, ws, B, H, W, expected_grad):
    lib = _lib()
    L.check(lib.ynet_conv2d_winograd_pred_bce_blob(src[0], src[2], u.data_ptr(), bias.data_ptr() if bias is not None else None, pred_wp.data_ptr(),
                                                   pred_bias.data_ptr() if pred_bias is not None else None, pred_cout, pos.data_ptr(), tmpl.blob.data_ptr(),
                                                   tmpl.blob.shape[0], tmpl.size, logits.data_ptr(), loss.data_ptr(), dx.data_ptr(), 32 * H * W, ws.data_ptr(), B, H, W,
                                                   expected_grad, _stream()), lib)


def conv2d_winograd_split_raw(src, u, dst0, dst0_s2d, dst1, cin, B, H, W):
    lib = _lib()
    L.check(lib.ynet_conv2d_winograd_split(src[0], src[1], u.data_ptr(), dst0[0], dst0[1], 1 if dst0_s2d else 0, dst1[0], dst1[1], cin, B, H, W, _stream()), lib)


def conv2d_winograd_cat_raw(srcs, u, bias, dst, B, H, W, relu, addend=None, pool=None, wbits_out=None, pool_code=None):
    lib = _lib()
    sp, sc, sb = _arrays(srcs)
    b = bias.data_ptr() if bias is not None else None
    if wbits_out is not None:
        if pool is not None or not relu:
            raise ValueError("conv2d_winograd_cat_raw: wbits_out is for a ReLU launch without the pooled copy")
        L.check(lib.ynet_conv2d_winograd_cat_relu_bits(sp, sc, sb, len(srcs), u.data_ptr(), b, dst[0], dst[1], B, H, W, addend[0] if addend else None,
                                                       addend[1] if addend else 0, addend[2] if addend else 0, wbits_out.data_ptr(), _stream()), lib)
        return
    if pool is not None and pool_code is not None:
        if not relu:
            raise ValueError("conv2d_winograd_cat_raw: pool_code is for a ReLU launch")
        L.check(lib.ynet_conv2d_winograd_cat_pool_code(sp, sc, sb, len(srcs), u.data_ptr(), b, dst[0], dst[1], pool[0], pool[1], pool_code.data_ptr(), B, H, W,
                                                       _stream()), lib)
        return
    if pool is not None:
        L.check(lib.ynet_conv2d_winograd_cat_pool(sp, sc, sb, len(srcs), u.data_ptr(), b, dst[0], dst[1], pool[0], pool[1], 32, B, H, W,
                                                  1 if relu else 0, _stream()), lib)
    elif addend is None:
        L.check(lib.ynet_conv2d_winograd_cat(sp, sc, sb, len(srcs), u.data_ptr(), b, dst[0], dst[1], 32, B, H, W, 1 if relu else 0, _stream()), lib)
    else:
        L.check(lib.ynet_conv2d_winograd_cat_add(sp, sc, sb, len(srcs), u.data_ptr(), b, dst[0], dst[1], 32, B, H, W, 1 if relu else 0,
                                                 addend[0], addend[1], addend[2], _stream()), lib)


_pool_code_allowed = _os.environ.get("YNET_POOL_CODE", "1") != "0"
_wino_relu_bits_allowed = _os.environ.get("YNET_WINOGRAD_RELU_BITS", "1") != "0"
_wino16_allowed = _os.environ.get("YNET_WINOGRAD16", "1") != "0"
_wino16_for_16 = _os.environ.get("YNET_WINOGRAD16_SLICE16", "0") != "0"
_split48_allowed = _os.environ.get("YNET_WINOGRAD_SPLIT48", "1") != "0"


def conv2d_winograd16_raw(srcs, u, bias, dst, cout, B, H, W, relu, relu_of=None, addend=None, pool=None):
    lib = _lib()
    sp, sc, sb = _arrays(srcs)
    L.check(lib.ynet_conv2d_winograd16(sp, sc, sb, len(srcs), u.data_ptr(), bias.data_ptr() if bias is not None else None, dst[0], dst[1], cout, B, H, W,
                                       1 if relu else 0, relu_of[0] if relu_of else None, relu_of[1] if relu_of else 0,
                                       addend[0] if addend else None, addend[1] if addend else 0, addend[2] if addend else 0,
                                       pool[0] if pool else None, pool[1] if pool else 0, _stream()), lib)


def _wino16_supported(srcs_c, cout, B, H, W, K=3):
    if not (_wino16_allowed and _wino_allowed and K == 3 and 1 <= len(srcs_c) <= 3):
        return False
    return bool(_lib().ynet_conv2d_winograd16_supported(B, H, W, (ctypes.c_int * len(srcs_c))(*srcs_c), len(srcs_c), cout, K))


def _wino16_filter(wino, wp, row0, cs, cout, col0, ctot):
    lib = _lib()
    cache, what = wino
    key = "wino16_%s_%d_%d_%d" % (what, row0, col0, cout)
    ent = cache.get(key)
    if ent is None or ent[0] is not wp or ent[2] != cs:
        ca = (ctypes.c_int * len(cs))(*cs)
        u = torch.empty(lib.ynet_winograd16_filter_floats(ca, len(cs), cout), device=wp.device, dtype=torch.float32)
        cols_pad = -(-ctot // 64) * 64
        L.check(lib.ynet_winograd16_filter(wp.data_ptr() + 4 * row0 * 9 * cols_pad, u.data_ptr(), ca, len(cs), cout, col0, ctot, _stream()), lib)
        ent = cache[key] = _wino_made((wp, u, cs))
    _wino_ready(ent)
    return ent


def _wino16(wino, wp, row0, srcs, bias, dst, cout, col0, ctot, B, H, W, relu, relu_of=None, addend=None, pool=None):
    ent = _wino16_filter(wino, wp, row0, tuple(s_[1] for s_ in srcs), cout, col0, ctot)
    conv2d_winograd16_raw(srcs, ent[1], None if bias is None else bias[col0:col0 + cout], dst, cout, B, H, W, relu, relu_of=relu_of, addend=addend, pool=pool)
    wino_stats["launches"] += 1
    wino_stats["launches16"] = wino_stats.get("launches16", 0) + 1


def _pad4(c):
    return (c + 3) & ~3


conv_auto = _os.environ.get("YNET_CONV_AUTO", "1") != "0"
_AUTO_TAG_CAT = {10: ("winograd_cat:2,3", "winograd_cat:2,6|code"), 40: ("winograd_cat:2,2", "winograd_cat:2,5|wbits"), 41: ("winograd_cat:2,0", "winograd_cat:2,4|wbits"),
                 30: ("winograd_cat:2,2", "winograd_cat:2,5|wbits")}


def _auto_tag(tk):
    if tk.family == 0:
        return None
    if tk.family == 1:
        return "winograd:" + "+".join("%d,%d,%d" % tuple(tk.tmpl[i]) for i in range(tk.nlaunch)) + ("|wbits" if tk.wrote_wbits else "")
    if tk.family == 2:
        return _AUTO_TAG_CAT[tk.variant][1 if (tk.wrote_wbits or tk.wrote_pool_code) else 0]
    if tk.family == 3:
        return "winograd16:" + "+".join("%d" % tk.tmpl[i][0] for i in range(tk.nlaunch))
    return "winograd_up:%d" % tk.family


def _auto_flags(wino):
    flags = 0
    if wino is None or not _wino_allowed:
        flags |= L.AUTO_NO_WINOGRAD
    if not _wino16_allowed:
        flags |= L.AUTO_NO_WINOGRAD16
    if _wino16_for_16:
        flags |= L.AUTO_WINOGRAD16_FOR_16
    if not _pool_code_allowed:
        flags |= L.AUTO_NO_POOL_CODE
    if not _split48_allowed:
        flags |= L.AUTO_NO_SPLIT48
    return flags


def conv2d_auto_raw(srcs, mask, wp, bias, dsts, B, H, W, K, relu, relu_of=None, pooled=None, bits_out=None, relu_bits=None, wino=None, wbits_out=None,
                    relu_wbits=None, pool_code=None, addend=None, upsample2x=False, wp_version=1, dst_s2d=None):
    lib = _lib()
    d = L.ConvAuto()
    d.nsrc, d.ndst = len(srcs), len(dsts)
    for i, s_ in enumerate(srcs):
        d.src[i], d.src_c[i], d.src_bs[i] = s_[0], s_[1], s_[2]
        d.src_bmod[i] = s_[3] if len(s_) > 3 else 0
    for i, t_ in enumerate(dsts):
        d.dst[i], d.dst_c[i], d.dst_bs[i] = t_[0], t_[1], t_[2]
        if dst_s2d is not None and dst_s2d[i]:
            d.dst_s2d[i] = 1
    if mask:
        d.mask, d.mask_bs = mask[0], mask[1]
    d.wp, d.bias = wp.data_ptr(), (bias.data_ptr() if bias is not None else None)
    d.B, d.H, d.W, d.K, d.relu, d.upsample2x = B, H, W, K, 1 if relu else 0, 1 if upsample2x else 0
    if relu_of is not None:
        d.relu_of, d.relu_of_bs = relu_of[0], relu_of[1]
    if pooled is not None:
        d.pooled, d.pooled_bs = pooled[0], pooled[1]
        if pool_code is not None:
            d.pool_code = pool_code.data_ptr()
    if addend is not None:
        d.addend, d.addend_bs, d.addend_bmod = addend[0], addend[1], addend[2]
    d.bits_out, d.relu_bits = bits_out, relu_bits
    if wbits_out is not None:
        d.wbits_out = wbits_out.data_ptr()
    if relu_wbits is not None:
        d.relu_wbits = relu_wbits.data_ptr()
    d.flags = flags = _auto_flags(wino)
    ent = None
    if wino is not None and not (flags & L.AUTO_NO_WINOGRAD):
        cache, what = wino
        need = lib.ynet_conv2d_auto_cache_floats(ctypes.byref(d))
        if need < 0:
            L.check(1, lib)
        if need > 0:
            key = "auto_" + what
            ent = cache.get(key)
            if ent is None or ent[0] is not wp or ent[1].numel() < need:
                ent = cache[key] = [wp, torch.empty(need, device=wp.device, dtype=torch.float32), (ctypes.c_ulonglong * 2)(0, 0), None, None]
            elif ent[4] is not None and not torch.cuda.is_current_stream_capturing():
                cur = torch.cuda.current_stream()
                if cur.cuda_stream != ent[3] and not ent[4].query():
                    cur.wait_event(ent[4])
            d.cache, d.cache_floats, d.cache_tag, d.wp_version = ent[1].data_ptr(), ent[1].numel(), ent[2], int(wp_version)
    if B * H * W <= 65536:
        nws = lib.ynet_conv2d_auto_workspace_floats(ctypes.byref(d))
        if nws > 0:
            key = (wp.device, torch.cuda.current_stream().cuda_stream)
            ws = _conv_ws.get(key)
            if ws is None or ws.numel() < nws:
                ws = _conv_ws[key] = torch.empty(nws, device=wp.device, dtype=torch.float32)
            d.workspace, d.workspace_floats = ws.data_ptr(), nws
    tk = L.ConvTaken()
    L.check(lib.ynet_conv2d_auto(ctypes.byref(d), ctypes.byref(tk), _stream()), lib)
    if tk.transformed and ent is not None and torch.cuda.is_available() and not torch.cuda.is_current_stream_capturing():
        ev = torch.cuda.Event()
        ev.record()
        ent[3], ent[4] = torch.cuda.current_stream().cuda_stream, ev
    if tk.family:
        wino_stats["launches"] += tk.nlaunch
        if tk.family in (3, 5):
            wino_stats["launches16"] = wino_stats.get("launches16", 0) + tk.nlaunch
    return _auto_tag(tk), tk


_dgrad_family_memo = {}


def dgrad_relu_family(B, H, W, dy_c, dx_c, K=3):
    key = (B, H, W, dy_c, dx_c, K, _wino_allowed, _wino16_allowed, _wino16_for_16)
    fam = _dgrad_family_memo.get(key)
    if fam is None:
        d, tk = L.ConvAuto(), L.ConvTaken()
        d.nsrc = d.ndst = 1
        d.src[0], d.src_c[0], d.src_bs[0] = 256, dy_c, dy_c * H * W
        d.dst[0], d.dst_c[0], d.dst_bs[0] = 256, dx_c, dx_c * H * W
        d.relu_of, d.relu_of_bs = 256, dx_c * H * W
        d.wp = 256
        d.B, d.H, d.W, d.K = B, H, W, K
        d.flags = (0 if _wino_allowed else L.AUTO_NO_WINOGRAD) | (0 if _wino16_allowed else L.AUTO_NO_WINOGRAD16) | (L.AUTO_WINOGRAD16_FOR_16 if _wino16_for_16 else 0)
        lib = _lib()
        L.check(lib.ynet_conv2d_auto_plan(ctypes.byref(d), ctypes.byref(tk)), lib)
        fam = _dgrad_family_memo[key] = int(tk.family)
    return fam


def conv2d_raw(srcs, mask, wp, bias, dsts, B, H, W, K, relu, relu_of=None, pooled=None, bits_out=None, relu_bits=None, wino=None, wbits_out=None,
               relu_wbits=None, pool_code=None, dst_s2d=None, info=None):
    if not conv_auto:
        return _conv2d_raw_py(srcs, mask, wp, bias, dsts, B, H, W, K, relu, relu_of=relu_of, pooled=pooled, bits_out=bits_out, relu_bits=relu_bits, wino=wino,
                              wbits_out=wbits_out, relu_wbits=relu_wbits, pool_code=pool_code, dst_s2d=dst_s2d, info=info)
    if wino is not None and not torch.is_grad_enabled() and (
            H * W < _wino_eval_min_hw or not (_wino_plain_eval if len(srcs) == 1 and srcs[0][1] in (16, 32) else _wino_cat_eval)):
        wino = None
    tag, tk = conv2d_auto_raw(srcs, mask, wp, bias, dsts, B, H, W, K, relu, relu_of=relu_of, pooled=pooled, bits_out=bits_out, relu_bits=relu_bits, wino=wino,
                              wbits_out=wbits_out, relu_wbits=relu_wbits, pool_code=pool_code, dst_s2d=dst_s2d)
    if info is not None:
        info["wrote_s2d"] = int(tk.wrote_s2d)
    return tag


def _conv2d_raw_py(srcs, mask, wp, bias, dsts, B, H, W, K, relu, relu_of=None, pooled=None, bits_out=None, relu_bits=None, wino=None, wbits_out=None,
                   relu_wbits=None, pool_code=None, dst_s2d=None, info=None):
    lib = _lib()
    sp, sc, sb = _arrays(srcs)
    if info is not None:
        info["wrote_s2d"] = 0
    if wino is not None and not torch.is_grad_enabled() and (
            H * W < _wino_eval_min_hw or not (_wino_plain_eval if len(srcs) == 1 and srcs[0][1] in (16, 32) else _wino_cat_eval)):
        wino = None
    if bits_out is not None:
        if len(dsts) != 1 or mask is not None or relu_of is not None or pooled is not None or not relu or _bmods(srcs) is not None:
            raise ValueError("conv2d_raw: bits_out is for a forward ReLU convolution with one destination")
        L.check(lib.ynet_conv2d_relu_bits(sp, sc, sb, len(srcs), wp.data_ptr(), bias.data_ptr() if bias is not None else None,
                                          dsts[0][0], dsts[0][1], dsts[0][2], bits_out, B, H, W, K, _stream()), lib)
        return
    if relu_bits is not None:
        if len(srcs) != 1 or len(dsts) != 1 or bias is not None or relu or relu_of is not None:
            raise ValueError("conv2d_raw: relu_bits is for a data gradient with one source and one destination")
        L.check(lib.ynet_conv2d_dgrad_relu_bits(srcs[0][0], srcs[0][1], srcs[0][2], mask[0] if mask else None, mask[1] if mask else 0,
                                                wp.data_ptr(), dsts[0][0], dsts[0][1], dsts[0][2], relu_bits, B, H, W, K, _stream()), lib)
        return
    if pooled is not None:
        if len(dsts) != 1 or mask is not None or relu_of is not None or _bmods(srcs) is not None:
            raise ValueError("conv2d_raw: pooled is for a forward convolution with one destination")
        if (wino is not None and _wino_allowed and K == 3 and dsts[0][1] == 32 and dsts[0][0] % 8 == 0 and dsts[0][2] % 2 == 0
                and all(len(s_) == 3 and s_[0] % 16 == 0 and s_[2] % 4 == 0 for s_ in srcs)):
            cs = (ctypes.c_int * len(srcs))(*[s_[1] for s_ in srcs])
            if lib.ynet_conv2d_winograd_cat_supported(B, H, W, cs, len(srcs), 32, K):
                cache, what = wino
                key = "wino_cat_" + what
                ent = cache.get(key)
                if ent is None or ent[0] is not wp or ent[2] != tuple(cs):
                    u = torch.empty(lib.ynet_winograd_filter_cat_floats(cs, len(srcs), 32), device=wp.device, dtype=torch.float32)
                    L.check(lib.ynet_winograd_filter_cat(wp.data_ptr(), u.data_ptr(), cs, len(srcs), 32, 0, 32, _stream()), lib)
                    ent = cache[key] = _wino_made((wp, u, tuple(cs)))
                _wino_ready(ent)
                code = pool_code if (relu and _pool_code_allowed) else None
                conv2d_winograd_cat_raw(srcs, ent[1], bias, (dsts[0][0], dsts[0][2]), B, H, W, relu, pool=pooled, pool_code=code)
                wino_stats["launches"] += 1
                return "winograd_cat:2,6|code" if code is not None else "winograd_cat:2,3"
        if (wino is not None and K == 3 and dsts[0][0] % 8 == 0 and dsts[0][2] % 2 == 0 and all(len(s_) == 3 and s_[0] % 16 == 0 and s_[2] % 4 == 0 for s_ in srcs)
                and _wino16_supported([s_[1] for s_ in srcs], dsts[0][1], B, H, W)):
            _wino16(wino, wp, 0, srcs, bias, (dsts[0][0], dsts[0][2]), dsts[0][1], 0, dsts[0][1], B, H, W, relu, pool=pooled)
            return "winograd16:3"
        L.check(lib.ynet_conv2d_pool(sp, sc, sb, len(srcs), wp.data_ptr(), bias.data_ptr() if bias is not None else None,
                                     dsts[0][0], dsts[0][1], dsts[0][2], pooled[0], pooled[1], B, H, W, K, 1 if relu else 0, _stream()), lib)
        return
    if (wino is not None and _wino_allowed and K == 3 and mask is None and len(srcs) == 1 and len(srcs[0]) == 3
            and srcs[0][0] % 16 == 0 and srcs[0][2] % 4 == 0 and (relu_of is None or (relu_of[0] % 8 == 0 and relu_of[1] % 2 == 0))):
        cin, ctot, HW = srcs[0][1], sum(d[1] for d in dsts), H * W
        pieces, piece_dst, c0 = [], [], 0
        for di, (ptr, c, bs) in enumerate(dsts):
            if ptr is None:
                c0 += c
                continue
            o = 0
            while c - o >= 16 and (c - o) % 16 == 0:
                n = 32 if c - o >= 32 else 16
                pieces.append((ptr + 4 * o * HW, n, bs, c0 + o))
                piece_dst.append((di, n == c))
                o += n
            if o != c:
                pieces = None
                break
            c0 += c
        if (_wino16_for_16 and pieces and len(pieces) == 1 and pieces[0][1] == 16 and pieces[0][0] % 8 == 0 and pieces[0][2] % 2 == 0
                and _wino16_supported([cin], 16, B, H, W)):
            ptr, n, bs, col0 = pieces[0]
            _wino16(wino, wp, 0, srcs, bias, (ptr, bs), 16, col0, ctot, B, H, W, relu, relu_of=relu_of)
            return "winograd16:%d" % (1 if relu_of is not None else 0)
        wide = any(d_[0] is not None and d_[1] >= 64 for d_ in dsts)
        if (_split48_allowed and pieces and not wide and len(pieces) == 2 and relu_of is None and bias is None and not relu and pieces[0][1] == 16 and piece_dst[0][1]
                and pieces[1][1] == 32 and piece_dst[1][1] and pieces[1][3] == pieces[0][3] + 16 and all(p_[0] % 8 == 0 and p_[2] % 2 == 0 for p_ in pieces)
                and all(lib.ynet_conv2d_winograd_supported(B, H, W, cin, p_[1], K) for p_ in pieces) and lib.ynet_conv2d_winograd_split_supported(B, H, W, cin)):
            cache, what = wino
            col0 = pieces[0][3]
            key = "wino_%s_%d_48" % (what, col0)
            ent = cache.get(key)
            if ent is None or ent[0] is not wp:
                ent = cache[key] = _wino_made((wp, winograd_filter(wp, cin, 48, col0, ctot)))
            _wino_ready(ent)
            s2d = bool(dst_s2d and dst_s2d[piece_dst[0][0]])
            conv2d_winograd_split_raw((srcs[0][0], srcs[0][2]), ent[1], (pieces[0][0], pieces[0][2]), s2d, (pieces[1][0], pieces[1][2]), cin, B, H, W)
            if s2d and info is not None:
                info["wrote_s2d"] |= 1 << piece_dst[0][0]
            wino_stats["launches"] += 1
            return "winograd:3,%d,%d" % (cin // 8, 6 if s2d else 5)
        if (pieces and not wide and len(pieces) <= (2 if relu_of is None else 1) and all(p_[0] % 8 == 0 and p_[2] % 2 == 0 for p_ in pieces)
                and all(lib.ynet_conv2d_winograd_supported(B, H, W, cin, p_[1], K) for p_ in pieces)):
            cache, what = wino
            one32 = len(pieces) == 1 and pieces[0][1] == 32
            wb_out = wbits_out if (one32 and relu and relu_of is None) else None
            wb_in = relu_wbits if (one32 and relu_of is not None and not relu and bias is None) else None
            em = 3 if wb_out is not None else (2 if wb_in is not None else (1 if relu_of is not None else 0))
            s2ds = [bool(dst_s2d and dst_s2d[di] and whole and em == 0 and bias is None and not relu) for di, whole in piece_dst]
            tag = ("winograd:" + "+".join("%d,%d,%d" % (p_[1] // 16, cin // 8, 4 if f_ else em) for p_, f_ in zip(pieces, s2ds))
                   + ("|wbits" if wb_out is not None else ""))
            for (ptr, n, bs, col0), (di, whole), s2d in zip(pieces, piece_dst, s2ds):
                key = "wino_%s_%d_%d" % (what, col0, n)
                ent = cache.get(key)
                if ent is None or ent[0] is not wp:
                    ent = cache[key] = _wino_made((wp, winograd_filter(wp, cin, n, col0, ctot)))
                _wino_ready(ent)
                conv2d_winograd_raw((srcs[0][0], srcs[0][2]), ent[1], None if bias is None else bias[col0:col0 + n], (ptr, bs), cin, n, B, H, W, relu,
                                    relu_of=None if wb_in is not None else relu_of, wbits_out=wb_out, relu_wbits=wb_in, **({"s2d": True} if s2d else {}))
                if s2d and info is not None:
                    info["wrote_s2d"] |= 1 << di
                wino_stats["launches"] += 1
            return tag
        wanted, c0 = [], 0
# ... 330 lines not shown


def _skip_register(x: torch.Tensor):
    for k in [k for k, e in _skip_registry.items() if e.ref() is None or e.consumed]:
        del _skip_registry[k]
    e = _SkipEntry()
    e.ref, e.shape, e.stash, e.consumed = weakref.ref(x), tuple(x.shape), [], False
    _skip_registry[x.data_ptr()] = e


def _skip_entry(t: torch.Tensor):
    e = _skip_registry.get(t.data_ptr())
    if e is None:
        return None
    if e.ref() is None or e.shape != tuple(t.shape):
        del _skip_registry[t.data_ptr()]
        return None
    return e


class _Conv2dFn(torch.autograd.Function):
    @staticmethod
    def forward(ctx, meta, weight, bias, lora_a, lora_b, *srcs):
        relu, scale, cache = meta["relu"], meta.get("scale", 1.0), meta["cache"]
        _need_gpu(weight, "conv2d weight")
        cout, cin, k, _ = weight.shape
        if meta.get("bcast"):
            srcs = [s.expand(meta["batch"], -1, -1, -1) if f else s for s, f in zip(srcs, meta["bcast"])]
        descs, keep = [], []
        reps = meta.get("repeat") or [1] * len(srcs)
        for i, s in enumerate(srcs):
            t, c, bs = _plane_desc(s, f"conv2d input {i}")
            keep.append(t)
            if reps[i] > 1:
                if ctx.needs_input_grad[5 + i]:
                    raise NotImplementedError("conv2d: a batch-repeated input cannot receive a gradient")
                descs.append((t.data_ptr(), c, c * t.shape[2] * t.shape[3] if t.shape[0] == 1 else t.stride(0), t.shape[0]))
            else:
                descs.append((t.data_ptr(), c, bs))
        if len(descs) > MAX_SRC:
            raise ValueError(f"conv2d: at most {MAX_SRC} concatenated inputs (got {len(descs)})")
        if sum(d[1] for d in descs) != cin:
            raise ValueError(f"conv2d: inputs carry {sum(d[1] for d in descs)} channels, weight expects {cin}")
        B, _, H, W = keep[0].shape
        B = max(t.shape[0] * r for t, r in zip(keep, reps))
        for t, r in zip(keep, reps):
            if t.shape[0] * r != B and not (t.shape[0] > 1 and t.stride(0) == 0):
                raise ValueError(f"conv2d: inputs disagree on the batch size ({[tuple(q.shape) for q in keep]}, repeat {reps})")
        wp = _cached(cache, weight, lora_a, lora_b, scale, "fwd")
        y = torch.empty((B, cout, H, W), device=weight.device, dtype=torch.float32)
        b = bias.detach() if bias is not None else None
        pooled = None
        if (meta.get("pool") and _pool_epilogue_allowed and not meta.get("repeat") and H % 2 == 0 and W % 2 == 0
                and all(d[0] % 16 == 0 and d[2] % 4 == 0 for d in descs) and _lib().ynet_conv2d_pool_supported(B, H, W, cout, k)):
            pooled = torch.empty((B, cout, H // 2, W // 2), device=weight.device, dtype=torch.float32)
        bits = None
        consumer_wino = (isinstance(meta.get("bits"), int) and not isinstance(meta.get("bits"), bool) and bool(meta.get("wino")) and _wino_allowed and k == 3
                         and dgrad_relu_family(B, H, W, int(meta["bits"]), cout, k) != 0)
        if (meta.get("bits") and not consumer_wino and relu and premask and _relu_bits_allowed and pooled is None and not meta.get("repeat")
                and all(d[0] % 16 == 0 and d[2] % 4 == 0 for d in descs)):
            n_words = _lib().ynet_conv2d_relu_bits_words(B, H, W, cout, k)
            if n_words > 0:
                bits = torch.empty(n_words, device=weight.device, dtype=torch.int32)
        wbits = None
        if (consumer_wino and cout == 32 and relu and premask and _wino_relu_bits_allowed and pooled is None and not meta.get("repeat")
                and int(meta["bits"]) in (16, 32) and bool(_lib().ynet_conv2d_winograd_supported(B, H, W, int(meta["bits"]), 32, k))):
            n_words = _lib().ynet_winograd_relu_bits_words(B, H, W)
            if n_words > 0:
                wbits = torch.empty(n_words, device=weight.device, dtype=torch.int32)
        pcode = None
        if pooled is not None and relu and cout == 32 and _pool_code_allowed and any(ctx.needs_input_grad) and meta.get("wino"):
            pcode = torch.empty((B, cout, H // 2, W // 2), device=weight.device, dtype=torch.uint8)
        defer = bool(meta.get("defer") and _conv_pred_bce_allowed and premask and relu and pooled is None and bits is None and wbits is None and len(descs) == 1
                     and len(descs[0]) == 3 and (cin, cout, k) == (32, 32, 3) and lora_a is None and not any(ctx.needs_input_grad[1:5]) and ctx.needs_input_grad[5]
                     and meta.get("wino") and _wino_allowed and descs[0][0] % 16 == 0 and descs[0][2] % 4 == 0 and keep[0].shape[0] == B
                     and _lib().ynet_conv2d_winograd_pred_bce_supported(B, H, W, 32, 32, 1, 1))
        if defer:
            def run(descs=descs, wp=wp, b=b, y=y, dims=(B, H, W), cache=cache):
                conv2d_raw(descs, None, wp, b, [(y.data_ptr(), 32, 32 * dims[1] * dims[2])], dims[0], dims[1], dims[2], 3, True, wino=(cache, "fwd"))
            _deferred[y.data_ptr()] = {"ref": weakref.ref(y), "shape": tuple(y.shape), "run": run, "src": descs[0], "wp": wp, "bias": b, "cache": cache,
                                       "dims": (B, H, W), "keep": keep[0]}
            took = None
        else:
            took = conv2d_raw(descs, None, wp, b, [(y.data_ptr(), cout, cout * H * W)], B, H, W, k, relu,
                              pooled=None if pooled is None else (pooled.data_ptr(), cout * (H // 2) * (W // 2)),
                              bits_out=None if bits is None else bits.data_ptr(), wino=(cache, "fwd") if meta.get("wino") else None, wbits_out=wbits,
                              pool_code=pcode)
        if not (isinstance(took, str) and took.endswith("|wbits")):
            wbits = None
        if not (isinstance(took, str) and took.endswith("|code")):
            pcode = None
        if pooled is not None:
            for k_ in [k_ for k_, e_ in _pooled_outputs.items() if e_[0]() is None]:
                del _pooled_outputs[k_]
            _pooled_outputs[y.data_ptr()] = (weakref.ref(y), tuple(y.shape), pooled, pcode)
        ctx.meta = meta
        ctx.n_src = len(srcs)
        ctx.has_bias = bias is not None
        ctx.has_lora = lora_a is not None
        ctx.save_for_backward(weight, lora_a, lora_b, y if relu else None, *keep)
        ctx.w_key = _weight_key(weight, lora_a, lora_b)
        if relu and premask:
            _relu_outputs[y.data_ptr()] = (weakref.ref(y), tuple(y.shape), bits, k, wbits)
        return y

    @staticmethod
    def backward(ctx, dy):
        weight, lora_a, lora_b, y, *srcs = ctx.saved_tensors
        meta = ctx.meta
        relu, scale, cache = meta["relu"], meta.get("scale", 1.0), meta["cache"]
        cout, cin, k, _ = weight.shape
        dy = dy.contiguous()
        B, _, H, W = dy.shape
        mask = (y.data_ptr(), cout * H * W) if relu else None
        if relu and _premasked:
            if _premasked.pop(dy.data_ptr(), None) == (y.data_ptr(), dy._version, tuple(dy.shape)):
                mask = None
                premask_stats["unmasked_backwards"] += 1
        if relu and mask is not None and _unmaterialized.get(y.data_ptr()) == tuple(y.shape):
            raise RuntimeError("conv2d backward: this convolution ran inside the fused predictor + criterion launch (its output was never written), but the gradient that "
                               "arrived does not carry its ReLU backward -- the output has another consumer, or a hook replaced its gradient: set YNET_CONV_PRED_BCE=0")
        need = ctx.needs_input_grad
        need_src = list(need[5:5 + ctx.n_src])
        d_srcs = [None] * ctx.n_src
        branch = None
        if (wgrad_branch and ctx.has_lora and dy.is_cuda and not need[1] and not (ctx.has_bias and need[2]) and (need[3] or need[4])
                and lora_a.is_leaf and lora_b.is_leaf and not lora_a._backward_hooks and not lora_b._backward_hooks
                and not getattr(lora_a, "_post_accumulate_grad_hooks", None) and not getattr(lora_b, "_post_accumulate_grad_hooks", None)):
            cur = torch.cuda.current_stream(dy.device)
            bkey, branch = _wgrad_stream(dy.device)
            branch.wait_stream(cur)
        if any(need_src) and meta.get("input_grad") is not None:
            if ctx.w_key != _weight_key(weight, lora_a, lora_b):
                raise RuntimeError("conv2d backward: a parameter was modified in place between forward and backward")
            d_srcs = _input_grad_srcs(meta, dy, y, _cached(cache, weight, lora_a, lora_b, scale, "dgrad"), srcs, need_src)
        elif any(need_src):
            if ctx.w_key != _weight_key(weight, lora_a, lora_b):
                raise RuntimeError("conv2d backward: a parameter was modified in place between forward and backward")
            wp_d = _cached(cache, weight, lora_a, lora_b, scale, "dgrad")
            dsts, want_s2d = [], []
            for i, s in enumerate(srcs):
                c = s.shape[1]
                if need_src[i]:
                    d_srcs[i] = torch.empty((B, c, H, W), device=dy.device, dtype=torch.float32)
                    dsts.append((d_srcs[i].data_ptr(), c, c * H * W))
                    w_ = _s2d_wanted.get(s.data_ptr()) if (premask and _upconv_s2d_allowed) else None
                    want_s2d.append(bool(w_ is not None and w_[0]() is not None and w_[1] == tuple(s.shape) and c == 16 and H % 2 == 0 and W % 2 == 0))
                else:
                    dsts.append((None, c, 0))
                    want_s2d.append(False)
            s2d_info = {} if any(want_s2d) else None
            s0 = srcs[0]
            emask = None
            if (premask and ctx.n_src == 1 and need_src[0] and _is_relu_output(s0) and s0.is_contiguous() and s0.shape[0] == B
                    and s0.data_ptr() % 16 == 0 and dy.data_ptr() % 16 == 0 and not (skip_fold and _skip_entry(s0) is not None)
                    and _lib().ynet_conv2d_dgrad_relu_supported(B, H, W, int(s0.shape[1]), int(k))):
                emask = (s0.data_ptr(), s0.shape[1] * H * W)
            ebits = None
            if emask is not None:
                e0 = _relu_outputs.get(s0.data_ptr())
                if (e0 is not None and e0[2] is not None and e0[3] == k and d_srcs[0].data_ptr() % 16 == 0
                        and _lib().ynet_conv2d_relu_bits_words(B, H, W, int(s0.shape[1]), int(k)) == e0[2].numel()):
                    ebits = e0[2]
            wino_em = (emask is not None and mask is None and bool(meta.get("wino")) and _wino_allowed and k == 3 and dy.data_ptr() % 16 == 0
                       and d_srcs[0].data_ptr() % 8 == 0 and s0.data_ptr() % 8 == 0 and dgrad_relu_family(B, H, W, cout, int(s0.shape[1]), int(k)) != 0)
            ewbits = None
            if wino_em and _wino_relu_bits_allowed and int(s0.shape[1]) == 32:
                e0 = _relu_outputs.get(s0.data_ptr())
                if (e0 is not None and len(e0) > 4 and e0[4] is not None and e0[4].numel() == _lib().ynet_winograd_relu_bits_words(B, H, W)
                        and _lib().ynet_conv2d_winograd_supported(B, H, W, cout, 32, int(k))):
# ... 1313 lines not shown
```

Baseline: 4978 trajectories/s.

## Compute batch-shared scene channels' convolution once and add it in pooled epilogue

When the first concatenated input has batch stride zero (the scene features are the same for every sample), its convolution contribution is computed once for a single image into a cached shared term. A second Winograd cat kernel then convolves only the per-sample channels and adds the shared term in a new pooled/code epilogue variant (EPI 7). This removes redundant per-batch convolution of the scene channels. In exchange it adds an extra launch and extra loads of the additive term in the epilogue.

```diff
diff --git a/include/ynet_hip.h b/include/ynet_hip.h
--- a/include/ynet_hip.h
+++ b/include/ynet_hip.h
@@ -64,6 +64,9 @@
                                   long long dst_bs, float* pooled, long long pooled_bs, int cout, int B, int H, int W, int relu, void* stream);
 int ynet_conv2d_winograd_cat_pool_code(const float* const* src, const int* src_c, const long long* src_bs, int nsrc, const float* u, const float* bias, float* dst,
                                        long long dst_bs, float* pooled, long long pooled_bs, unsigned char* code, int B, int H, int W, void* stream);
+int ynet_conv2d_winograd_cat_add_pool_code(const float* const* src, const int* src_c, const long long* src_bs, int nsrc, const float* u, const float* bias, float* dst,
+                                           long long dst_bs, float* pooled, long long pooled_bs, unsigned char* code, int B, int H, int W, const float* addend,
+                                           long long addend_bs, int addend_bmod, void* stream);
 long long ynet_winograd_relu_bits_words(int B, int H, int W);
 int ynet_conv2d_winograd_relu_bits(const float* src, long long src_bs, const float* u, const float* bias, float* dst, long long dst_bs, int cin, int B, int H, int W,
                                    unsigned* bits_out, void* stream);
@@ -89,6 +92,7 @@
 #define YNET_AUTO_NO_RELU_WBITS 16u
 #define YNET_AUTO_NO_SPLIT48 32u
 #define YNET_AUTO_UPCONV_BWD 64u
+#define YNET_AUTO_NO_SHARED_SCENE 128u
 typedef struct YnetConvAuto {
     const float* src[4];
     int src_c[4];
@@ -125,6 +129,7 @@
     long long workspace_floats;
     unsigned flags;
     int dst_s2d[4];
+    float* shared_term;
 } YnetConvAuto;
 typedef struct YnetConvTaken {
     int family;
diff --git a/motion-style-transfer_amd/_lib.py b/motion-style-transfer_amd/_lib.py
--- a/motion-style-transfer_amd/_lib.py
+++ b/motion-style-transfer_amd/_lib.py
@@ -23,7 +23,7 @@
                 ("addend", c_fp), ("addend_bs", c_ll), ("addend_bmod", c_i),
                 ("bits_out", c_fp), ("relu_bits", c_fp), ("wbits_out", c_fp), ("relu_wbits", c_fp),
                 ("cache", c_fp), ("cache_floats", c_ll), ("cache_tag", ctypes.POINTER(ctypes.c_ulonglong)), ("wp_version", ctypes.c_ulonglong),
-                ("workspace", c_fp), ("workspace_floats", c_ll), ("flags", ctypes.c_uint), ("dst_s2d", c_i * 4)]
+                ("workspace", c_fp), ("workspace_floats", c_ll), ("flags", ctypes.c_uint), ("dst_s2d", c_i * 4), ("shared_term", c_fp)]
 
 
 class ConvTaken(ctypes.Structure):
@@ -32,6 +32,7 @@
 
 
 AUTO_NO_WINOGRAD, AUTO_NO_WINOGRAD16, AUTO_WINOGRAD16_FOR_16, AUTO_NO_POOL_CODE, AUTO_NO_RELU_WBITS, AUTO_NO_SPLIT48 = 1, 2, 4, 8, 16, 32
+AUTO_NO_SHARED_SCENE = 128
 AUTO_UPCONV_BWD = 64
 
 SIGNATURES = {
@@ -70,6 +71,7 @@
     "ynet_conv2d_winograd_cat_add": (c_i, [PP, PI, PLL, c_i, c_fp, c_fp, c_fp, c_ll, c_i, c_i, c_i, c_i, c_i, c_fp, c_ll, c_i, c_fp]),
     "ynet_conv2d_winograd_cat_pool": (c_i, [PP, PI, PLL, c_i, c_fp, c_fp, c_fp, c_ll, c_fp, c_ll, c_i, c_i, c_i, c_i, c_i, c_fp]),
     "ynet_conv2d_winograd_cat_pool_code": (c_i, [PP, PI, PLL, c_i, c_fp, c_fp, c_fp, c_ll, c_fp, c_ll, c_fp, c_i, c_i, c_i, c_fp]),
+    "ynet_conv2d_winograd_cat_add_pool_code": (c_i, [PP, PI, PLL, c_i, c_fp, c_fp, c_fp, c_ll, c_fp, c_ll, c_fp, c_i, c_i, c_i, c_fp, c_ll, c_i, c_fp]),
     "ynet_winograd_relu_bits_words": (c_ll, [c_i, c_i, c_i]),
     "ynet_conv2d_winograd_relu_bits": (c_i, [c_fp, c_ll, c_fp, c_fp, c_fp, c_ll, c_i, c_i, c_i, c_i, c_fp, c_fp]),
     "ynet_conv2d_winograd_cat_relu_bits": (c_i, [PP, PI, PLL, c_i, c_fp, c_fp, c_fp, c_ll, c_i, c_i, c_i, c_fp, c_ll, c_i, c_fp, c_fp]),
diff --git a/motion-style-transfer_amd/csrc/conv_auto.cpp b/motion-style-transfer_amd/csrc/conv_auto.cpp
--- a/motion-style-transfer_amd/csrc/conv_auto.cpp
+++ b/motion-style-transfer_amd/csrc/conv_auto.cpp
@@ -123,6 +123,15 @@
     if (a->pooled) {
         YNET_REQUIRE(a->ndst == 1 && !a->mask && !a->relu_of, "conv2d_auto: pooled is for a forward convolution with one destination");
         const bool okp = wino && srcs_aligned(a) && al(a->dst[0], 8) && !(a->dst_bs[0] & 1) && a->nsrc <= 3;
+        if (okp && ctot == 32 && a->shared_term && !(a->flags & (YNET_AUTO_NO_SHARED_SCENE | YNET_AUTO_NO_POOL_CODE)) && a->pool_code && a->relu && a->nsrc >= 2 && B > 1 &&
+            a->src_bs[0] == 0 && al(a->shared_term, 8) && ynet_conv2d_winograd_cat_supported(B, H, W, cs, a->nsrc, 32, K) &&
+            ynet_conv2d_winograd_cat_supported(B, H, W, cs + 1, a->nsrc - 1, 32, K) && cs[0] > 4 && cs[0] <= 56) {
+            p.family = 2;
+            p.variant = 13;
+            add_launch(p, K_CAT, 0, cs, 1, 32, 0, 32);
+            add_launch(p, K_CAT, cs[0], cs + 1, a->nsrc - 1, 32, 0, 32);
+            return 0;
+        }
         if (okp && ctot == 32 && ynet_conv2d_winograd_cat_supported(B, H, W, cs, a->nsrc, 32, K)) {
             p.family = 2;
             p.variant = 10;
@@ -463,6 +472,17 @@
             if (wb) return done(ynet_conv2d_winograd_cat_relu_bits(a->src, a->src_c, a->src_bs, a->nsrc, u0, a->bias, a->dst[0], a->dst_bs[0], B, H, W, a->addend, a->addend_bs, a->addend_bmod, wb, stream));
             return done(ynet_conv2d_winograd_cat_add(a->src, a->src_c, a->src_bs, a->nsrc, u0, a->bias, a->dst[0], a->dst_bs[0], 32, B, H, W, relu, a->addend, a->addend_bs, a->addend_bmod, stream));
         }
+        if (p.variant == 13) {
+            const long long HW = (long long)H * W;
+            const long long zero = 0;
+            int rc = ynet_conv2d_winograd_cat(a->src, a->src_c, &zero, 1, u0, a->bias, a->shared_term, 32 * HW, 32, 1, H, W, 0, stream);
+            if (rc) return rc;
+            tag(0, 2, 0, 0);
+            tag(1, 2, 7, 0);
+            t.wrote_pool_code = 1;
+            return done(ynet_conv2d_winograd_cat_add_pool_code(a->src + 1, a->src_c + 1, a->src_bs + 1, a->nsrc - 1, u1, nullptr, a->dst[0], a->dst_bs[0], a->pooled, a->pooled_bs,
+                                                               a->pool_code, B, H, W, a->shared_term, 32 * HW, 1, stream));
+        }
         if (p.variant == 10) {
             unsigned char* code = (relu && !(a->flags & YNET_AUTO_NO_POOL_CODE)) ? a->pool_code : nullptr;
             tag(0, 2, code ? 6 : 3, 0);
diff --git a/motion-style-transfer_amd/csrc/conv_wino.hip b/motion-style-transfer_amd/csrc/conv_wino.hip
--- a/motion-style-transfer_amd/csrc/conv_wino.hip
+++ b/motion-style-transfer_amd/csrc/conv_wino.hip
@@ -54,10 +54,11 @@
     return r;
 }
 
-template <int NCB, int EPI, int BITS = 0, bool S2D = false, int CB0 = 0, int CB1 = NCB>
-__device__ __forceinline__ void wino_epilogue(f32x4 (&acc)[16][NCB], const f32x2 (&bias2)[NCB][2], float floor_v, __amdgpu_buffer_rsrc_t ry,
-                                              __amdgpu_buffer_rsrc_t rm, unsigned st0, unsigned st1, unsigned so_t, unsigned sm_t, int HW, unsigned stp = 0,
-                                              unsigned* wbits = nullptr, unsigned char* pcode = nullptr) {
+template <int NCB, int EPI, int BITS, bool S2D, int CB0, int CB1, bool ADDP>
+__device__ __forceinline__ void wino_epilogue_impl(f32x4 (&acc)[16][NCB], const f32x2 (&bias2)[NCB][2], float floor_v, __amdgpu_buffer_rsrc_t ry,
+                                                   __amdgpu_buffer_rsrc_t rm, unsigned st0, unsigned st1, unsigned so_t, unsigned sm_t, int HW, unsigned stp,
+                                                   unsigned* wbits, unsigned char* pcode, __amdgpu_buffer_rsrc_t rad, unsigned sad_t) {
+    static_assert(!ADDP || EPI == 3, "ADDP is the pooled epilogue with an additive term");
     unsigned word = 0u;
     if constexpr (BITS == 2) word = *wbits;
 #pragma unroll
@@ -65,6 +66,16 @@
         constexpr int NB = CB1 - CB0;
         const int cd = cb - CB0;
         u32x2 mk[2][2][2];
+        if constexpr (ADDP) {
+#pragma unroll
+            for (int h = 0; h < 2; ++h)
+#pragma unroll
+                for (int k = 0; k < 2; ++k) {
+                    const unsigned sm = sad_t + (unsigned)((cd * 16 + 2 * h + k) * HW * 4);
+                    mk[h][k][0] = __builtin_amdgcn_raw_buffer_load_b64(rad, st0, sm, 0);
+                    mk[h][k][1] = __builtin_amdgcn_raw_buffer_load_b64(rad, st1, sm, 0);
+                }
+        }
         if constexpr (EPI == 1 || EPI == 2) {
 #pragma unroll
             for (int h = 0; h < 2; ++h)
@@ -93,7 +104,7 @@
 #pragma unroll
             for (int k = 0; k < 2; ++k) {
                 f32x2 row0 = {o00[k], o01[k]}, row1 = {o10[k], o11[k]};
-                if constexpr (EPI == 2) {
+                if constexpr (EPI == 2 || ADDP) {
                     row0 += __builtin_bit_cast(f32x2, mk[h][k][0]);
                     row1 += __builtin_bit_cast(f32x2, mk[h][k][1]);
                 }
@@ -147,6 +158,13 @@
     if constexpr (BITS == 1) *wbits = word;
 }
 
+template <int NCB, int EPI, int BITS = 0, bool S2D = false, int CB0 = 0, int CB1 = NCB>
+__device__ __forceinline__ void wino_epilogue(f32x4 (&acc)[16][NCB], const f32x2 (&bias2)[NCB][2], float floor_v, __amdgpu_buffer_rsrc_t ry,
+                                              __amdgpu_buffer_rsrc_t rm, unsigned st0, unsigned st1, unsigned so_t, unsigned sm_t, int HW, unsigned stp = 0,
+                                              unsigned* wbits = nullptr, unsigned char* pcode = nullptr) {
+    wino_epilogue_impl<NCB, EPI, BITS, S2D, CB0, CB1, false>(acc, bias2, floor_v, ry, rm, st0, st1, so_t, sm_t, HW, stp, wbits, pcode, ry, 0u);
+}
+
 template <int MB, typename PosT>
 __device__ __forceinline__ float wino_epilogue_pred(f32x4 (&acc)[16][2], const f32x2 (&bias2)[2][2], const f32x4* tab,
                                                     const WinoArgs& a, __amdgpu_buffer_rsrc_t rdx, __amdgpu_buffer_rsrc_t rlog, unsigned st_rm, unsigned so_rm, int b,
@@ -578,9 +596,10 @@
 
 template <int NCB, int EPI_>
 __global__ __launch_bounds__(WN_THREADS, 1) void conv_wino_cat_kernel(const WinoCatArgs a) {
-    constexpr int EPI = EPI_ == 4 ? 0 : (EPI_ == 5 ? 2 : (EPI_ == 6 ? 3 : EPI_));
-    constexpr int BITS = EPI_ == 6 ? 3 : (EPI_ >= 4 ? 1 : 0);
+    constexpr int EPI = EPI_ == 4 ? 0 : (EPI_ == 5 ? 2 : (EPI_ == 6 || EPI_ == 7 ? 3 : EPI_));
+    constexpr int BITS = EPI_ == 6 || EPI_ == 7 ? 3 : (EPI_ >= 4 ? 1 : 0);
     constexpr bool ADD = EPI == 2;
+    constexpr bool ADDP = EPI_ == 7;
     extern __shared__ f32x4 smem[];
     constexpr int WQ = 4 * NCB * 64;
     const int tid = threadIdx.x, lane = tid & 63;
@@ -710,7 +729,10 @@
                          : __builtin_amdgcn_make_buffer_rsrc(const_cast<float*>(ADD ? a.addend + (long long)ab * a.addend_bs : a.y), 0, y_img, 0x00020000);
             unsigned* wb = BITS == 1 ? a.wbits + (((long long)b * (H >> 1) + (ty * (WN_TH / 2) + (cur & 7))) * tiles_x + tx) * 64 + lane : nullptr;
             unsigned char* pc = BITS == 3 ? a.pcode + ((long long)b * (16 * NCB) * (HW >> 2) + ((stp + sa_t) >> 2)) : nullptr;
-            wino_epilogue<NCB, EPI, BITS>(acc, bias2, floor_v, ry, ra, st0, st1, so_t, sa_t, HW, stp, wb, pc);
+            if constexpr (ADDP) {
+                const __amdgpu_buffer_rsrc_t rad = __builtin_amdgcn_make_buffer_rsrc(const_cast<float*>(a.addend + (long long)ab * a.addend_bs), 0, y_img, 0x00020000);
+                wino_epilogue_impl<NCB, 3, 3, false, 0, NCB, true>(acc, bias2, floor_v, ry, ra, st0, st1, so_t, sa_t, HW, stp, wb, pc, rad, so_t);
+            } else wino_epilogue<NCB, EPI, BITS>(acc, bias2, floor_v, ry, ra, st0, st1, so_t, sa_t, HW, stp, wb, pc);
         }
         cur = nxt;
         if (cur < total_units) nxt = next_unit();
@@ -1343,7 +1365,7 @@
     return n;
 }
 
-static bool wino_cat_ok(int B, int H, int W, const int* src_c, int nsrc, int cout, int K) {
+static bool wino_cat_shape_ok(int B, int H, int W, const int* src_c, int nsrc, int cout, int K) {
     static const int on = getenv("YNET_WINOGRAD") ? atoi(getenv("YNET_WINOGRAD")) : 1;
     static const int cat_on = getenv("YNET_WINOGRAD_CAT") ? atoi(getenv("YNET_WINOGRAD_CAT")) : 1;
     if (!on || !cat_on || K != 3 || B <= 0 || nsrc < 1 || nsrc > WC_MAX_SRC || cout != 32) return false;
@@ -1352,7 +1374,11 @@
         if (src_c[i] <= 0) return false;
     const int nch = wino_cat_padded(src_c, nsrc) / 4;
     if (56ll * H * W * 4 + (W + 4) * 4 >= (1ll << 31)) return false;
-    if (nch < 2 || nch > 14) return false;
+    return nch >= 2 && nch <= 14;
+}
+
+static bool wino_cat_ok(int B, int H, int W, const int* src_c, int nsrc, int cout, int K) {
+    if (!wino_cat_shape_ok(B, H, W, src_c, nsrc, cout, K)) return false;
     static const int min_pixels = getenv("YNET_WINOGRAD_MIN") ? atoi(getenv("YNET_WINOGRAD_MIN")) : 128 * 128 * 8;
     return (long long)B * H * W >= min_pixels;
 }
@@ -1382,7 +1408,7 @@
                            long long dst_bs, int cout, int B, int H, int W, int relu, const float* addend, long long addend_bs, int addend_bmod, float* pool,
                            long long pool_bs, void* stream, const char* what, unsigned* wbits = nullptr, unsigned char* pcode = nullptr) {
     YNET_REQUIRE(src && src_c && src_bs && u && dst, "%s: null pointer", what);
-    YNET_REQUIRE(wino_cat_ok(B, H, W, src_c, nsrc, cout, 3), "%s: shape B=%d %dx%d -> %d with %d sources is not served (ask ynet_conv2d_winograd_cat_supported)", what,
+    YNET_REQUIRE(wino_cat_shape_ok(B, H, W, src_c, nsrc, cout, 3), "%s: shape B=%d %dx%d -> %d with %d sources is not served (ask ynet_conv2d_winograd_cat_supported)", what,
                  B, H, W, cout, nsrc);
     const long long HW = (long long)H * W;
     WinoCatArgs a{};
@@ -1400,8 +1426,8 @@
                      "%s: the additive term must be 8-byte aligned, its image stride not smaller than the image, its modulus not negative", what);
     }
     if (pool != nullptr)
-        YNET_REQUIRE(addend == nullptr && (reinterpret_cast<uintptr_t>(pool) & 3) == 0 && pool_bs >= cout * (HW / 4),
-                     "%s: the pooled copy must have a batch stride not smaller than its image, and excludes an additive term", what);
+        YNET_REQUIRE((addend == nullptr || pcode != nullptr) && (reinterpret_cast<uintptr_t>(pool) & 3) == 0 && pool_bs >= cout * (HW / 4),
+                     "%s: the pooled copy must have a batch stride not smaller than its image, and takes an additive term only together with the code bytes", what);
     if (wbits != nullptr)
         YNET_REQUIRE(pool == nullptr && (reinterpret_cast<uintptr_t>(wbits) & 3) == 0, "%s: the 1-bit mask excludes the pooled copy and must be 4-byte aligned", what);
     if (pcode != nullptr) YNET_REQUIRE(pool != nullptr && cout == 32 && relu, "%s: the arg-max / ReLU bytes come with the pooled copy of a 32-channel ReLU output", what);
@@ -1431,6 +1457,7 @@
         (void)hipFuncSetAttribute(reinterpret_cast<const void*>(conv_wino_cat_kernel<2, 4>), hipFuncAttributeMaxDynamicSharedMemorySize, 14 * 8192 + 8 * WC_RING_BYTES + 16);
         (void)hipFuncSetAttribute(reinterpret_cast<const void*>(conv_wino_cat_kernel<2, 5>), hipFuncAttributeMaxDynamicSharedMemorySize, 14 * 8192 + 8 * WC_RING_BYTES + 16);
         (void)hipFuncSetAttribute(reinterpret_cast<const void*>(conv_wino_cat_kernel<2, 6>), hipFuncAttributeMaxDynamicSharedMemorySize, 14 * 8192 + 8 * WC_RING_BYTES + 16);
+        (void)hipFuncSetAttribute(reinterpret_cast<const void*>(conv_wino_cat_kernel<2, 7>), hipFuncAttributeMaxDynamicSharedMemorySize, 14 * 8192 + 8 * WC_RING_BYTES + 16);
         int dev = 0, cus = 256;
         (void)hipGetDevice(&dev);
         (void)hipDeviceGetAttribute(&cus, hipDeviceAttributeMultiprocessorCount, dev);
@@ -1439,7 +1466,8 @@
     }
     int grid = a.ntiles < cus_dev[slot] ? a.ntiles : cus_dev[slot];
     if (grid >= 8) grid &= ~7;
-    if (wbits != nullptr && addend != nullptr) hipLaunchKernelGGL((conv_wino_cat_kernel<2, 5>), dim3(grid), dim3(WN_THREADS), lds, (hipStream_t)stream, a);
+    if (pcode != nullptr && addend != nullptr) hipLaunchKernelGGL((conv_wino_cat_kernel<2, 7>), dim3(grid), dim3(WN_THREADS), lds, (hipStream_t)stream, a);
+    else if (wbits != nullptr && addend != nullptr) hipLaunchKernelGGL((conv_wino_cat_kernel<2, 5>), dim3(grid), dim3(WN_THREADS), lds, (hipStream_t)stream, a);
     else if (wbits != nullptr) hipLaunchKernelGGL((conv_wino_cat_kernel<2, 4>), dim3(grid), dim3(WN_THREADS), lds, (hipStream_t)stream, a);
     else if (addend != nullptr) hipLaunchKernelGGL((conv_wino_cat_kernel<2, 2>), dim3(grid), dim3(WN_THREADS), lds, (hipStream_t)stream, a);
     else if (pcode != nullptr) hipLaunchKernelGGL((conv_wino_cat_kernel<2, 6>), dim3(grid), dim3(WN_THREADS), lds, (hipStream_t)stream, a);
@@ -1471,6 +1499,14 @@
     YNET_REQUIRE(pooled != nullptr && code != nullptr, "conv2d_winograd_cat_pool_code: the pooled output or its code plane is null");
     return wino_cat_launch(src, src_c, src_bs, nsrc, u, bias, dst, dst_bs, 32, B, H, W, 1, nullptr, 0, 0, pooled, pooled_bs, stream, "conv2d_winograd_cat_pool_code",
                            nullptr, code);
+}
+
+int ynet_conv2d_winograd_cat_add_pool_code(const float* const* src, const int* src_c, const long long* src_bs, int nsrc, const float* u, const float* bias, float* dst,
+                                           long long dst_bs, float* pooled, long long pooled_bs, unsigned char* code, int B, int H, int W, const float* addend,
+                                           long long addend_bs, int addend_bmod, void* stream) {
+    YNET_REQUIRE(pooled != nullptr && code != nullptr && addend != nullptr, "conv2d_winograd_cat_add_pool_code: the pooled output, its code plane or the additive term is null");
+    return wino_cat_launch(src, src_c, src_bs, nsrc, u, bias, dst, dst_bs, 32, B, H, W, 1, addend, addend_bs, addend_bmod, pooled, pooled_bs, stream,
+                           "conv2d_winograd_cat_add_pool_code", nullptr, code);
 }
 
 static int wino_launch_any(const float* src, long long src_bs, const float* u, const float* bias, float* dst, long long dst_bs, const float* emask,
diff --git a/motion-style-transfer_amd/ops.py b/motion-style-transfer_amd/ops.py
--- a/motion-style-transfer_amd/ops.py
+++ b/motion-style-transfer_amd/ops.py
@@ -390,6 +390,10 @@
     if pool is not None and pool_code is not None:
         if not relu:
             raise ValueError("conv2d_winograd_cat_raw: pool_code is for a ReLU launch")
+        if addend is not None:
+            L.check(lib.ynet_conv2d_winograd_cat_add_pool_code(sp, sc, sb, len(srcs), u.data_ptr(), b, dst[0], dst[1], pool[0], pool[1], pool_code.data_ptr(), B, H, W,
+                                                               addend[0], addend[1], addend[2], _stream()), lib)
+            return
         L.check(lib.ynet_conv2d_winograd_cat_pool_code(sp, sc, sb, len(srcs), u.data_ptr(), b, dst[0], dst[1], pool[0], pool[1], pool_code.data_ptr(), B, H, W,
                                                        _stream()), lib)
         return
@@ -403,6 +407,8 @@
                                                  addend[0], addend[1], addend[2], _stream()), lib)
 
 
+_shared_scene_allowed = _os.environ.get("YNET_SHARED_SCENE", "1") != "0"
+shared_scene_stats = {"launches": 0}
 _pool_code_allowed = _os.environ.get("YNET_POOL_CODE", "1") != "0"
 _wino_relu_bits_allowed = _os.environ.get("YNET_WINOGRAD_RELU_BITS", "1") != "0"
 _wino16_allowed = _os.environ.get("YNET_WINOGRAD16", "1") != "0"
@@ -453,7 +459,7 @@
 
 conv_auto = _os.environ.get("YNET_CONV_AUTO", "1") != "0"
 _AUTO_TAG_CAT = {10: ("winograd_cat:2,3", "winograd_cat:2,6|code"), 40: ("winograd_cat:2,2", "winograd_cat:2,5|wbits"), 41: ("winograd_cat:2,0", "winograd_cat:2,4|wbits"),
-                 30: ("winograd_cat:2,2", "winograd_cat:2,5|wbits")}
+                 30: ("winograd_cat:2,2", "winograd_cat:2,5|wbits"), 13: ("winograd_cat:2,0+2,7|code", "winograd_cat:2,0+2,7|code")}
 
 
 def _auto_tag(tk):
@@ -480,11 +486,13 @@
         flags |= L.AUTO_NO_POOL_CODE
     if not _split48_allowed:
         flags |= L.AUTO_NO_SPLIT48
+    if not _shared_scene_allowed:
+        flags |= L.AUTO_NO_SHARED_SCENE
     return flags
 
 
 def conv2d_auto_raw(srcs, mask, wp, bias, dsts, B, H, W, K, relu, relu_of=None, pooled=None, bits_out=None, relu_bits=None, wino=None, wbits_out=None,
-                    relu_wbits=None, pool_code=None, addend=None, upsample2x=False, wp_version=1, dst_s2d=None):
+                    relu_wbits=None, pool_code=None, addend=None, upsample2x=False, wp_version=1, dst_s2d=None, shared_term=None):
     lib = _lib()
     d = L.ConvAuto()
     d.nsrc, d.ndst = len(srcs), len(dsts)
@@ -507,6 +515,8 @@
             d.pool_code = pool_code.data_ptr()
     if addend is not None:
         d.addend, d.addend_bs, d.addend_bmod = addend[0], addend[1], addend[2]
+    if shared_term is not None:
+        d.shared_term = shared_term.data_ptr()
     d.bits_out, d.relu_bits = bits_out, relu_bits
     if wbits_out is not None:
         d.wbits_out = wbits_out.data_ptr()
@@ -520,7 +530,7 @@
         if need < 0:
             L.check(1, lib)
         if need > 0:
-            key = "auto_" + what
+            key = "auto_" + what + ("_shared" if shared_term is not None else "")
             ent = cache.get(key)
             if ent is None or ent[0] is not wp or ent[1].numel() < need:
                 ent = cache[key] = [wp, torch.empty(need, device=wp.device, dtype=torch.float32), (ctypes.c_ulonglong * 2)(0, 0), None, None]
@@ -545,6 +555,8 @@
         ent[3], ent[4] = torch.cuda.current_stream().cuda_stream, ev
     if tk.family:
         wino_stats["launches"] += tk.nlaunch
+        if tk.variant == 13:
+            shared_scene_stats["launches"] += 1
         if tk.family in (3, 5):
             wino_stats["launches16"] = wino_stats.get("launches16", 0) + tk.nlaunch
     return _auto_tag(tk), tk
@@ -572,22 +584,44 @@
 
 
 def conv2d_raw(srcs, mask, wp, bias, dsts, B, H, W, K, relu, relu_of=None, pooled=None, bits_out=None, relu_bits=None, wino=None, wbits_out=None,
-               relu_wbits=None, pool_code=None, dst_s2d=None, info=None):
+               relu_wbits=None, pool_code=None, dst_s2d=None, info=None, shared_term=None):
     if not conv_auto:
         return _conv2d_raw_py(srcs, mask, wp, bias, dsts, B, H, W, K, relu, relu_of=relu_of, pooled=pooled, bits_out=bits_out, relu_bits=relu_bits, wino=wino,
-                              wbits_out=wbits_out, relu_wbits=relu_wbits, pool_code=pool_code, dst_s2d=dst_s2d, info=info)
+                              wbits_out=wbits_out, relu_wbits=relu_wbits, pool_code=pool_code, dst_s2d=dst_s2d, info=info, shared_term=shared_term)
     if wino is not None and not torch.is_grad_enabled() and (
             H * W < _wino_eval_min_hw or not (_wino_plain_eval if len(srcs) == 1 and srcs[0][1] in (16, 32) else _wino_cat_eval)):
         wino = None
     tag, tk = conv2d_auto_raw(srcs, mask, wp, bias, dsts, B, H, W, K, relu, relu_of=relu_of, pooled=pooled, bits_out=bits_out, relu_bits=relu_bits, wino=wino,
-                              wbits_out=wbits_out, relu_wbits=relu_wbits, pool_code=pool_code, dst_s2d=dst_s2d)
+                              wbits_out=wbits_out, relu_wbits=relu_wbits, pool_code=pool_code, dst_s2d=dst_s2d, shared_term=shared_term)
     if info is not None:
         info["wrote_s2d"] = int(tk.wrote_s2d)
     return tag
 
 
+def conv2d_shared_scene_raw(srcs, wp, bias, dst, pooled, pool_code, shared_term, B, H, W, wino):
+    lib = _lib()
+    cache, what = wino
+    cs = tuple(s_[1] for s_ in srcs)
+    key = "wino_cat_shared_" + what
+    ent = cache.get(key)
+    if ent is None or ent[0] is not wp or ent[3] != cs:
+        c0, cr = (ctypes.c_int * 1)(cs[0]), (ctypes.c_int * (len(cs) - 1))(*cs[1:])
+        u0 = torch.empty(lib.ynet_winograd_filter_cat_floats(c0, 1, 32), device=wp.device, dtype=torch.float32)
+        u1 = torch.empty(lib.ynet_winograd_filter_cat_floats(cr, len(cs) - 1, 32), device=wp.device, dtype=torch.float32)
+        L.check(lib.ynet_winograd_filter_cat(wp.data_ptr(), u0.data_ptr(), c0, 1, 32, 0, 32, _stream()), lib)
+        L.check(lib.ynet_winograd_filter_cat(wp.data_ptr() + 4 * cs[0] * 9 * 64, u1.data_ptr(), cr, len(cs) - 1, 32, 0, 32, _stream()), lib)
+        ent = cache[key] = _wino_made((wp, u0, u1, cs))
+    _wino_ready(ent)
+    term = (shared_term.data_ptr(), 32 * H * W)
+    conv2d_winograd_cat_raw([(srcs[0][0], srcs[0][1], 0)], ent[1], bias, term, 1, H, W, False)
+    conv2d_winograd_cat_raw(srcs[1:], ent[2], None, dst, B, H, W, True, addend=term + (1,), pool=pooled, pool_code=pool_code)
+    wino_stats["launches"] += 2
+    shared_scene_stats["launches"] += 1
+    return "winograd_cat:2,0+2,7|code"
+
+
 def _conv2d_raw_py(srcs, mask, wp, bias, dsts, B, H, W, K, relu, relu_of=None, pooled=None, bits_out=None, relu_bits=None, wino=None, wbits_out=None,
-                   relu_wbits=None, pool_code=None, dst_s2d=None, info=None):
+                   relu_wbits=None, pool_code=None, dst_s2d=None, info=None, shared_term=None):
     lib = _lib()
     sp, sc, sb = _arrays(srcs)
     if info is not None:
@@ -613,6 +647,11 @@
         if (wino is not None and _wino_allowed and K == 3 and dsts[0][1] == 32 and dsts[0][0] % 8 == 0 and dsts[0][2] % 2 == 0
                 and all(len(s_) == 3 and s_[0] % 16 == 0 and s_[2] % 4 == 0 for s_ in srcs)):
             cs = (ctypes.c_int * len(srcs))(*[s_[1] for s_ in srcs])
+            if (shared_term is not None and _shared_scene_allowed and relu and pool_code is not None and _pool_code_allowed and len(srcs) >= 2 and B > 1
+                    and srcs[0][2] == 0 and 4 < srcs[0][1] <= 56 and shared_term.data_ptr() % 8 == 0
+                    and lib.ynet_conv2d_winograd_cat_supported(B, H, W, cs, len(srcs), 32, K)
+                    and lib.ynet_conv2d_winograd_cat_supported(B, H, W, (ctypes.c_int * (len(srcs) - 1))(*cs[1:]), len(srcs) - 1, 32, K)):
+                return conv2d_shared_scene_raw(srcs, wp, bias, (dsts[0][0], dsts[0][2]), pooled, pool_code, shared_term, B, H, W, wino)
             if lib.ynet_conv2d_winograd_cat_supported(B, H, W, cs, len(srcs), 32, K):
                 cache, what = wino
                 key = "wino_cat_" + what
@@ -1109,10 +1148,16 @@
                                        "dims": (B, H, W), "keep": keep[0]}
             took = None
         else:
+            more = {}
+            if pcode is not None and _shared_scene_allowed and len(descs) >= 2 and len(descs[0]) == 3 and descs[0][2] == 0 and B > 1 and keep[0].shape[0] == B:
+                tkey = "shared_term_%dx%d" % (H, W)
+                if tkey not in cache:
+                    cache[tkey] = torch.empty((1, cout, H, W), device=weight.device, dtype=torch.float32)
+                more["shared_term"] = cache[tkey]
             took = conv2d_raw(descs, None, wp, b, [(y.data_ptr(), cout, cout * H * W)], B, H, W, k, relu,
                               pooled=None if pooled is None else (pooled.data_ptr(), cout * (H // 2) * (W // 2)),
                               bits_out=None if bits is None else bits.data_ptr(), wino=(cache, "fwd") if meta.get("wino") else None, wbits_out=wbits,
-                              pool_code=pcode)
+                              pool_code=pcode, **more)
         if not (isinstance(took, str) and took.endswith("|wbits")):
             wbits = None
         if not (isinstance(took, str) and took.endswith("|code")):
```

After: 4969 trajectories/s. No clear change (-0.2%).
